# audiocogs/aac.js

Hardware: AMD Instinct MI355X
Metric: AAC-LC 48 kHz stereo frames/sec per node + achieved HBM GB/s vs roofline (higher is better)
Workload: dtype f32

## Files before the change

aac.js_amd/csrc/aacg_device.h:

```cpp
#ifndef AACG_DEVICE_H
#define AACG_DEVICE_H

#include <stdint.h>
#include "../../include/aacgpu.h"
#include "../../include/aacgpu_tools.h"

#define AACG_RUN_W        AACG_RUN_FRAMES
#define AACG_WG_WAVES     AACG_RUN_W
#define AACG_WG_THREADS   (AACG_WG_WAVES * 64)

#define AACG_PCM_SCALE (1.0f / 32768.0f)

struct aacg_c2 { float re, im; };

struct aacg_tables {
    aacg_c2 sincos_long[8][64];
    aacg_c2 tw512[7][64];
    aacg_c2 tw64[7][8];
    aacg_c2 sincos_short[8][8];
    float win_long[2][1024];
    float win_short[2][128];
    float sf[432];
    float iq_signed[1024];
    uint8_t band_of_long[1024];
    uint8_t band_of_short[128];
    float iq[8192];
};

#define AACG_TAB_OFF_SINCOS_LONG  0
#define AACG_TAB_OFF_TW512        (AACG_TAB_OFF_SINCOS_LONG + 8 * 64 * 2)
#define AACG_TAB_OFF_TW64         (AACG_TAB_OFF_TW512 + 7 * 64 * 2)
#define AACG_TAB_OFF_SINCOS_SHORT (AACG_TAB_OFF_TW64 + 7 * 8 * 2)
#define AACG_TAB_OFF_WIN_LONG     (AACG_TAB_OFF_SINCOS_SHORT + 8 * 8 * 2)
#define AACG_TAB_OFF_WIN_SHORT    (AACG_TAB_OFF_WIN_LONG + 2 * 1024)
#define AACG_TAB_F32_FLOATS       (AACG_TAB_OFF_WIN_SHORT + 2 * 128)
#define AACG_TAB_OFF_SF           AACG_TAB_F32_FLOATS
#define AACG_TAB_OFF_IQ_SMALL     (AACG_TAB_OFF_SF + 432)
#define AACG_TAB_OFF_BAND_LONG    (AACG_TAB_OFF_IQ_SMALL + 1024)
#define AACG_TAB_OFF_BAND_SHORT   (AACG_TAB_OFF_BAND_LONG + 256)
#define AACG_TAB_QUANT_FLOATS     (AACG_TAB_OFF_BAND_SHORT + 32)

#define AACG_SLOT_FLOATS  2048
#define AACG_TAB_SLOT_BASE(tab_floats) (((tab_floats) + 127) & ~127)
#define AACG_LDS_FLOATS(tab_floats) (AACG_TAB_SLOT_BASE(tab_floats) + AACG_WG_WAVES * AACG_SLOT_FLOATS + AACG_WG_WAVES)
#define AACG_LDS_BYTES_F32    (4 * AACG_LDS_FLOATS(AACG_TAB_F32_FLOATS))
#define AACG_LDS_BYTES_QUANT  (4 * AACG_LDS_FLOATS(AACG_TAB_QUANT_FLOATS))

struct aacg_dev_unit {
    aacg_unit_desc d;
    uint32_t gmap[2];
    uint32_t cpl_first, cpl_n;
};

struct aacg_dev_tns {
    int32_t start[8];
    int32_t size[8];
    int32_t inc[8];
    int32_t order[8];
    float   lpc[8][AACG_TNS_MAX_ORDER];
};

struct aacg_pns_tables {
    float    rnd[1024];
    double   esum[1028];
    uint16_t swb_long[64];
    uint16_t swb_short[16];
};

#define AACG_OV_BUFFERS 16
#define AACG_PIPE_STREAMS 3

struct aacg_run {
    int32_t pred_unit;
    int32_t n_units;
    int32_t is_last;
    uint32_t wave_nch;
    int32_t ov0[2];
    int32_t rot[2];
    int32_t unit[AACG_RUN_W];
    int32_t  wave_unit[AACG_RUN_W];
    uint32_t wave_coef[AACG_RUN_W];
    uint32_t wave_meta[AACG_RUN_W];
};
static_assert(sizeof(aacg_run) == 288 && __builtin_offsetof(aacg_run, ov0) == 16 && __builtin_offsetof(aacg_run, wave_unit) == 96,
              "aacg_run: the header is read as eight dwords, the per-wave words by offset (imdct_run_body)");
static inline int32_t aacg_run_wave_unit(const aacg_run& r, int w)
{
    if (r.pred_unit >= 0 && w == 0) return r.pred_unit;
    const int k = (r.pred_unit >= 0 && r.n_units < AACG_RUN_W) ? w - 1 : w;
    return k < r.n_units ? r.unit[k] : -1;
}

struct aacg_couple_job {
    uint32_t cce_unit;
    uint32_t src, dst, stride;
    uint32_t gain_off;
    uint32_t reserved[3];
};

struct aacg_couple_params {
    const aacg_couple_job* jobs;
    const aacg_dev_unit*   units;
    const aacg_band_meta*  meta;
    const aacg_tables*     tab;
    const float*           gains;
    float*                 spec;
    const float*           side;
    float*                 pcm;
    int32_t                n_jobs;
    int32_t                reserved;
};

struct aacg_kparams {
    const aacg_dev_unit*  units;
    const aacg_run*       runs;
    const void*           coeffs;
    const aacg_band_meta* meta;
    const aacg_dev_tns*   tns;
    float*                pcm;
    float*                overlap;
    float*                spec_out;
    const aacg_tables*    tab;
    int32_t               flip;
    int32_t               n_runs;
    int32_t               ablate;
    int32_t               reserved;
    float*                scratch;
    const aacg_pns_tables* pns;
};
static inline void aacg_set_tns_m(aacg_kparams* P, const double* m) { P->scratch = (float*)(void*)m; }
static inline void aacg_set_cpl(aacg_kparams* P, const aacg_couple_job* jobs, const float* gains, const float* side)
{
    P->scratch = (float*)(void*)jobs; P->pns = (const aacg_pns_tables*)(const void*)gains; P->spec_out = (float*)side;
}
#define AACG_CPL_JOBS(P)  ((const aacg_couple_job*)(const void*)(P).scratch)
#define AACG_CPL_GAINS(P) ((const float*)(const void*)(P).pns)
#define AACG_CPL_SIDE(P)  ((const float*)(P).spec_out)

struct aacg_rv_link {
    int32_t link_in;
    int32_t link_out;
    int32_t succ_unit;
    int32_t reserved;
};
#define AACG_RV_STATE_WORDS 2
#define AACG_RV_DATA_FLOATS 4096
#define AACG_RV_TAIL 1ull
#define AACG_RV_HEAD 2ull

struct aacg_xl_cell {
    unsigned long long state;
    unsigned long long pcm;
    uint32_t n_out_ch;
    uint32_t reserved[3];
};
struct aacg_rv_args {
    const aacg_rv_link*  links;
    unsigned long long*  state;
    float*               data;
    unsigned long long   epoch;
    aacg_xl_cell*        xl_cells;
    float*               xl_head;
    unsigned long long   epoch_in;
};

#define AACG_PARSE_WG_SMALL   256
#define AACG_PARSE_WG_LARGE   1024
#define AACG_PARSE_L1_BITS    9
#define AACG_PARSE_LUT_WORDS  12288
#define AACG_PARSE_BUCKETS    1024
#define AACG_PARSE_PAD_BYTES  32
#define AACG_PARSE_LDS_FIXED(lut_words, threads) ((size_t)(lut_words) * 4u + 160u + (size_t)AACG_MAX_SECTIONS * (threads) + 16u)
typedef struct aacg_parse_tables {
    uint32_t lut[AACG_PARSE_LUT_WORDS];
    uint32_t lut_words;
    uint16_t swb_long[64];
    uint16_t swb_short[16];
    uint32_t n_swb_long, n_swb_short;
    float    tns_coef[4][16];
} aacg_parse_tables;

typedef struct aacg_parse_params {
    const uint32_t* bytes;
    const aacg_parse_frame* frames;
    const aacg_parse_tables* tab;
    aacg_unit_desc* units;
    int16_t* q;
    aacg_band_meta* meta;
    aacg_tns_info* tns;
    aacg_parse_result* results;
    uint32_t n_frames, max_units, max_channels, options;
    uint32_t arena_bytes;
    uint32_t wg_threads;
    const uint32_t* order;
} aacg_parse_params;

typedef struct aacg_walk_params {
    aacg_parse_params P;
    aacg_parse_frame* blocks;
    aacg_walk_result* results;
    uint32_t max_frames;
} aacg_walk_params;

#endif
```

aac.js_amd/csrc/aacg_engine.hip:

```cpp
#include <hip/hip_runtime.h>

#include <chrono>
#include <hip/hip_ext.h>

#include <cstdio>
#include <cstdlib>
#include <cstring>
#include <new>
#include <string>
#include <algorithm>
#include <vector>
#include <mutex>
#include <thread>
#include <unordered_map>
#include <sys/mman.h>

#include "aacg_kernels.h"
#include "aacg_host.h"
#include "aacg_routes.h"
#include "aacg_wait.h"

extern "C" __global__ __launch_bounds__(AACG_WG_THREADS)
void aacg_imdct_run_quant(const aacg_kparams P) { imdct_run_body<AACG_INPUT_QUANT_I16>(P); }

// ... 5 lines not shown
    {0, "aacg_imdct_run_f32", (const void*)aacg_imdct_run_f32}
};
const int aacg_run_kernels_plain_n = 2;

void aacg_refresh_launch(aacg_dev_unit* units, const aacg_unit_desc* parsed, aacg_parse_result* results, const aacg_refresh_map* map, uint32_t n_units,
                         uint32_t max_units, int refuse_pns, uint32_t* refused, hipStream_t s);
int aacg_spectral_ex_set_lds_limits(void);
void aacg_spectral_ex_launch(bool quant, int n_units, hipStream_t s, const aacg_kparams& P);
void aacg_tns_matrices_launch(const aacg_dev_tns* d_recs, double* d_m, uint32_t n_records, hipStream_t s);
void aacg_couple_launch(bool pcm, hipStream_t s, const aacg_couple_params& Q);
struct cce_bufs { const aacg_run* runs; const aacg_couple_job* jobs; const float* gains; float* side; };
struct rv_bufs { const aacg_run* runs; const aacg_rv_link* links; unsigned long long* state; float* data; };

extern "C" __global__ __launch_bounds__(AACG_WG_THREADS)
void aacg_spectral(const aacg_kparams P, int n_units) { spectral_body(P, n_units); }

extern "C" __global__ void aacg_probe_wait(const unsigned* flag, unsigned* seen, long long ticks)
{
    const long long t0 = wall_clock64();
    unsigned ok = 0;
    while (!ok && wall_clock64() - t0 < ticks) ok = __hip_atomic_load(flag, __ATOMIC_RELAXED, __HIP_MEMORY_SCOPE_AGENT);
    *seen = ok;
}
extern "C" __global__ void aacg_probe_set(unsigned* flag) { __hip_atomic_store(flag, 1u, __ATOMIC_RELAXED, __HIP_MEMORY_SCOPE_AGENT); }

#define AACG_LDS_BYTES_SPECTRAL ((AACG_TAB_QUANT_FLOATS + AACG_WG_WAVES * 512) * 4)

struct aacg_engine {
    aacg_config cfg;
    hipStream_t stream = nullptr;
    aacg_tables* d_tab = nullptr;
    aacg_pns_tables* d_pns = nullptr;
    unsigned long long rv_epoch = 0;
    float* d_overlap = nullptr;
    std::vector<uint8_t> parity;
    uint64_t epoch = 0;
    aacg_tables h_tab;
    aacg_host_windows h_win;
    struct pipe_t {
        hipStream_t stream[AACG_PIPE_STREAMS] = {};
        hipEvent_t mark[AACG_PIPE_RING][AACG_PIPE_STREAMS] = {};
        hipEvent_t seen[AACG_PIPE_RING][AACG_PIPE_STREAMS] = {};
        hipEvent_t tail[AACG_PIPE_STREAMS] = {};
        hipEvent_t fork = nullptr;
        uint64_t n = 0;
        int streams = AACG_PIPE_STREAMS;
        uint64_t issued = 0;
        hipStream_t joined_stream = nullptr; uint64_t joined_n = ~0ull;
        bool open = false;
        bool concurrent = false;
        bool serial = false;
        aacg_plan* plan = nullptr;
        unsigned long long epoch = 0;
        uint64_t chained = 0;
    } pipe;
    aacg_xl_cell* d_xl_cells = nullptr;
    float* d_xl_head = nullptr;
    struct slot_t {
        hipStream_t stream = nullptr;
        hipEvent_t done = nullptr, kernel_done = nullptr;
        bool busy = false;
        void* d_units = nullptr;  size_t units_cap = 0;
        void* d_runs = nullptr;   size_t runs_cap = 0;
        void* d_coeffs = nullptr; size_t coeffs_cap = 0;
        void* d_meta = nullptr;   size_t meta_cap = 0;
        void* d_tns = nullptr;    size_t tns_cap = 0;
        void* d_scratch = nullptr; size_t scratch_cap = 0;
        void* d_spec = nullptr;   size_t spec_cap = 0;
        void* d_cce[4] = {nullptr, nullptr, nullptr, nullptr}; size_t cce_cap[4] = {0, 0, 0, 0};
        void* d_rv[4] = {nullptr, nullptr, nullptr, nullptr}; size_t rv_cap[4] = {0, 0, 0, 0};
        void* d_pcm = nullptr;    size_t pcm_cap = 0;
        void* h_in = nullptr;     size_t h_in_cap = 0;
        void* h_pcm = nullptr;    size_t h_pcm_cap = 0;
        void* user_pcm = nullptr; size_t user_pcm_bytes = 0;
        aacg_plan_host h;
    } slot[2];
    std::vector<std::pair<void*, size_t>> pool;
    uint64_t submitted = 0;
    hipEvent_t last_kernel = nullptr;
    void* d_trace = nullptr;
    int debug_route = 0;
    int ablate = 0;
    aacg_wait_policy wait;
    std::vector<hipStream_t> foreign;
    float* h_ov = nullptr;
    bool wedged = false;
    hipStream_t dump_stream = nullptr;
    aacg_xl_cell* h_dump = nullptr;
    std::string pipe_note;
    std::string err;
};

#define AACG_PLAN_BUFFERS 13
struct aacg_plan {
    aacg_engine* e;
    aacg_plan_host h;
    uint32_t n_units = 0;
    aacg_dev_unit* d_units = nullptr;
    aacg_run* d_runs = nullptr;
    aacg_dev_tns* d_tns = nullptr;
    float* d_scratch = nullptr;
    float* d_spec = nullptr;
    void*  d_cce[4] = {nullptr, nullptr, nullptr, nullptr};
    void*  d_rv[4] = {nullptr, nullptr, nullptr, nullptr};
    size_t bytes[AACG_PLAN_BUFFERS] = {0, 0, 0, 0, 0, 0, 0, 0, 0, 0, 0, 0, 0};
    hipEvent_t uploaded = nullptr;
    hipEvent_t last_use = nullptr;
    hipStream_t last_stream = nullptr;
    uint32_t unit_sets = 1, cur_set = 0;
    const aacg_dev_unit* units_now() const { return d_units + (size_t)cur_set * n_units; }
    bool used = false;
    bool last_pipelined = false;
    uint64_t seen_epoch = ~0ull;
    uint32_t launches = 0;
};

namespace {

bool hip_ok(aacg_engine* e, hipError_t rc, const char* what)
{
    if (rc == hipSuccess) return true;
    if (e) e->err = std::string(what) + ": " + hipGetErrorString(rc);
    return false;
}

#define HIP_TRY(e, call, code) do { if (!hip_ok((e), (call), #call)) return (code); } while (0)

size_t coef_elem_size(const aacg_engine* e) { return e->cfg.input_kind == AACG_INPUT_QUANT_I16 ? 2 : 4; }
size_t pcm_elem_size(const aacg_engine* e) { return e->cfg.output_kind == AACG_OUTPUT_I16 ? 2 : 4; }

void* pool_take(aacg_engine* e, size_t bytes, size_t* got)
{
    size_t best = e->pool.size();
    for (size_t i = 0; i < e->pool.size(); i++)
        if (e->pool[i].second >= bytes && e->pool[i].second <= 2 * bytes + 4096 && (best == e->pool.size() || e->pool[i].second < e->pool[best].second)) best = i;
    if (best != e->pool.size()) {
        void* p = e->pool[best].first;
        *got = e->pool[best].second;
        e->pool.erase(e->pool.begin() + (long)best);
        return p;
    }
    void* p = nullptr;
    if (!hip_ok(e, hipMalloc(&p, bytes), "hipMalloc (plan)")) return nullptr;
    *got = bytes;
    return p;
}

void pool_give(aacg_engine* e, void* p, size_t bytes)
{
    if (!p) return;
    if (e->pool.size() >= 48) { (void)hipFree(e->pool.front().first); e->pool.erase(e->pool.begin()); }
    e->pool.emplace_back(p, bytes);
}

int grow(aacg_engine* e, void** p, size_t* cap, size_t need)
{
    if (need <= *cap) return AACG_OK;
    if (*p) { (void)hipFree(*p); *p = nullptr; *cap = 0; }
    HIP_TRY(e, hipMalloc(p, need), AACG_ERR_OUT_OF_MEMORY);
    *cap = need;
    return AACG_OK;
}

int grow_host(aacg_engine* e, void** p, size_t* cap, size_t need)
{
    if (need <= *cap) return AACG_OK;
    if (*p) { (void)hipHostFree(*p); *p = nullptr; *cap = 0; }
    HIP_TRY(e, hipHostMalloc(p, need, hipHostMallocDefault), AACG_ERR_OUT_OF_MEMORY);
    *cap = need;
    return AACG_OK;
}

bool is_pinned(const void* p)
{
    hipPointerAttribute_t a;
    if (hipPointerGetAttributes(&a, p) != hipSuccess) { (void)hipGetLastError(); return false; }
    return a.type == hipMemoryTypeHost;
}

#define AACG_DUMP_CELLS 4096u
const char* event_state(hipEvent_t ev)
{
    if (!ev) return "-";
    const hipError_t st = hipEventQuery(ev);
    (void)hipGetLastError();
    return st == hipSuccess ? "done" : st == hipErrorNotReady ? "PENDING" : "error";
}
const char* stream_state(hipStream_t s)
{
    const hipError_t st = hipStreamQuery(s);
    (void)hipGetLastError();
    return st == hipSuccess ? "idle" : st == hipErrorNotReady ? "BUSY" : "error";
}

std::string in_flight(aacg_engine* e)
{
    char b[512];
    std::string o;
    const aacg_engine::pipe_t& pp = e->pipe;
    std::snprintf(b, sizeof b, "pipeline: %llu launches issued, %llu in the current sequence on %d streams, %llu chained, open %d serial %d concurrent %d, rv epoch %llu; ",
                  (unsigned long long)pp.issued, (unsigned long long)pp.n, pp.streams, (unsigned long long)pp.chained, (int)pp.open, (int)pp.serial, (int)pp.concurrent, e->rv_epoch);
    o += b;
    o += std::string("engine stream ") + stream_state(e->stream);
    for (int k = 0; k < AACG_PIPE_STREAMS; k++) if (pp.stream[k]) { std::snprintf(b, sizeof b, ", pipe stream %d %s", k, stream_state(pp.stream[k])); o += b; }
    for (int k = 0; k < 2; k++) if (e->slot[k].stream) { std::snprintf(b, sizeof b, ", batch slot %d %s (busy %d, kernel %s, copy-back %s)", k, stream_state(e->slot[k].stream), (int)e->slot[k].busy, event_state(e->slot[k].kernel_done), event_state(e->slot[k].done)); o += b; }
    for (size_t k = 0; k < e->foreign.size(); k++) { std::snprintf(b, sizeof b, ", caller stream %p %s", (void*)e->foreign[k], stream_state(e->foreign[k])); o += b; }
    if (pp.stream[0]) {
        o += "; completion events [ring slot: per stream]";
        for (int r = 0; r < AACG_PIPE_RING; r++) {
            std::snprintf(b, sizeof b, " %d:", r); o += b;
            for (int k = 0; k < AACG_PIPE_STREAMS; k++) { o += k ? "/" : ""; o += event_state(pp.seen[r][k] ? pp.seen[r][k] : nullptr); }
        }
    }
    const size_t n_cells = (size_t)e->cfg.max_streams * (size_t)e->cfg.max_channels * (size_t)AACG_OV_BUFFERS;
    const size_t take = n_cells < AACG_DUMP_CELLS ? n_cells : AACG_DUMP_CELLS;
    if (!e->dump_stream && hipStreamCreateWithFlags(&e->dump_stream, hipStreamNonBlocking) != hipSuccess) { (void)hipGetLastError(); e->dump_stream = nullptr; }
    hipStream_t ds = e->dump_stream;
    aacg_xl_cell* h = e->h_dump;
    if (e->d_xl_cells && ds && h && hipMemcpyAsync(h, e->d_xl_cells, take * sizeof(aacg_xl_cell), hipMemcpyDeviceToHost, ds) == hipSuccess) {
        aacg_wait_policy quick; quick.limit_s = 0.25;
        if (aacg_wait_stream(ds, quick) == hipSuccess) {
            unsigned long long n_tail = 0, n_head = 0, lo = ~0ull, hi = 0;
            std::string heads;
            for (size_t i = 0; i < take; i++) {
                const unsigned long long w = h[i].state, ep = w >> 2;
                if (!w) continue;
                if ((w & 3) == AACG_RV_TAIL) n_tail++;
                if ((w & 3) == AACG_RV_HEAD) { n_head++; if (n_head <= 4) { std::snprintf(b, sizeof b, " cell %zu epoch %llu", i, ep); heads += b; } }
                lo = ep < lo ? ep : lo; hi = ep > hi ? ep : hi;
            }
            std::snprintf(b, sizeof b, "; cross-launch cells (first %zu of %zu): %llu TAIL, %llu HEAD (a HEAD nobody finished = a consumer whose producer never came:%s), epochs %llu..%llu",
                          take, n_cells, n_tail, n_head, heads.empty() ? " none" : heads.c_str(), lo == ~0ull ? 0ull : lo, hi);
            o += b;
        } else o += "; cross-launch cells unreadable: a device-to-host copy on a fresh stream did not complete in 250 ms either";
    } else { (void)hipGetLastError(); o += "; cross-launch cells not read"; }
    return o;
}

int timed_out(aacg_engine* e, const char* what)
{
    char b[160];
    std::snprintf(b, sizeof b, "%s: the GPU did not answer within %.1f s (aacg_set_wait_limit_ms). In flight: ", what, e->wait.limit_s);
    e->err = std::string(b) + in_flight(e);
    e->wedged = true;
    return AACG_ERR_TIMEOUT;
}
int wait_stream(aacg_engine* e, hipStream_t s, const char* what)
{
    const hipError_t st = aacg_wait_stream(s, e->wait);
    if (st == hipSuccess) return AACG_OK;
    if (st == hipErrorNotReady) return timed_out(e, what);
    e->err = std::string(what) + ": " + hipGetErrorString(st);
    return AACG_ERR_NO_DEVICE;
}
int wait_event(aacg_engine* e, hipEvent_t ev, const char* what)
{
    const hipError_t st = aacg_wait_event(ev, e->wait);
    if (st == hipSuccess) return AACG_OK;
    if (st == hipErrorNotReady) return timed_out(e, what);
    e->err = std::string(what) + ": " + hipGetErrorString(st);
    return AACG_ERR_NO_DEVICE;
}
void note_stream(aacg_engine* e, hipStream_t s)
{
    if (!s || s == e->stream) return;
    for (hipStream_t k : e->pipe.stream) if (k == s) return;
    for (hipStream_t k : e->foreign) if (k == s) return;
    if (e->foreign.size() >= 32) e->foreign.erase(e->foreign.begin());
    e->foreign.push_back(s);
}

}

const aacg_run_kernel* aacg_find_run_kernel(unsigned key)
{
    const aacg_run_kernel* const tabs[] = {aacg_run_kernels_plain, aacg_run_kernels_rv, aacg_run_kernels_nt, aacg_run_kernels_ext,
                                           aacg_run_kernels_i16, aacg_run_kernels_exrun, aacg_run_kernels_couple};
    const int counts[] = {aacg_run_kernels_plain_n, aacg_run_kernels_rv_n, aacg_run_kernels_nt_n, aacg_run_kernels_ext_n,
                          aacg_run_kernels_i16_n, aacg_run_kernels_exrun_n, aacg_run_kernels_couple_n};
    for (size_t t = 0; t < sizeof tabs / sizeof tabs[0]; t++)
        for (int i = 0; i < counts[t]; i++)
            if (tabs[t][i].key == key) return &tabs[t][i];
    return nullptr;
}

namespace {

aacg_route route_of(const aacg_engine* e, const aacg_plan_host& h, bool pipelined)
{
    return aacg_pick_route(e->cfg.input_kind, e->cfg.output_kind, e->debug_route, e->d_trace != nullptr, h, pipelined);
}

bool needs_spec_buffer(const aacg_engine* e, const aacg_plan_host& h) { return route_of(e, h, false).stage != AACG_STAGE_NONE; }

int launch_kernel(aacg_engine* e, const aacg_run_kernel* k, unsigned blocks, hipStream_t s, const aacg_kparams& P, const aacg_rv_args* V, hipEvent_t stop = nullptr)
{
    if (!k) { e->err = "no run kernel for this route"; return AACG_ERR_UNSUPPORTED; }
    aacg_kparams p = P;
    aacg_rv_args v;
    void* args[8] = {&p, nullptr, nullptr, nullptr, nullptr, nullptr, nullptr, nullptr};
    if (k->key & AACG_RK_RV) { v = *V; args[1] = &v; }
    const void *a_runs = p.runs, *a_tab = p.tab, *a_links = V ? V->links : nullptr, *a_units = p.units, *a_coeffs = p.coeffs, *a_meta = p.meta;
    if (k->preloaded) { args[0] = &a_runs; args[1] = &a_tab; args[2] = &a_links; args[3] = &a_units; args[4] = &a_coeffs; args[5] = &a_meta; args[6] = &p; args[7] = &v; }
    const dim3 block(AACG_WG_THREADS);
    if (stop) HIP_TRY(e, hipExtLaunchKernel(k->fn, dim3(blocks), block, args, 0, s, nullptr, stop, 0), AACG_ERR_NO_DEVICE);
    else      HIP_TRY(e, hipLaunchKernel(k->fn, dim3(blocks), block, args, 0, s), AACG_ERR_NO_DEVICE);
    return AACG_OK;
}

static size_t tns_record_bytes(size_t n) { return (sizeof(aacg_dev_tns) * n + 255u) & ~(size_t)255u; }
static size_t tns_buffer_bytes(size_t n) { return n ? tns_record_bytes(n) + sizeof(double) * AACG_TNS_M_DOUBLES * n : 0; }
static double* tns_matrices_of(const aacg_dev_tns* d_tns, size_t n) { return (double*)((char*)const_cast<aacg_dev_tns*>(d_tns) + tns_record_bytes(n)); }

struct xl_args { bool on; unsigned long long epoch_in; int set; int trace_part = 0; };

int launch_run(aacg_engine* e, const aacg_route& R, const aacg_dev_unit* d_units, const aacg_run* d_runs, const aacg_dev_tns* d_tns,
               float* d_scratch, float* d_spec, const cce_bufs& cb, const rv_bufs& rvb, const aacg_plan_host& h, const void* d_coeffs, const aacg_band_meta* d_meta,
               void* d_pcm, int flip, hipStream_t s, const xl_args& xl, unsigned long long* epoch_out, hipEvent_t stop = nullptr)
{
    if (h.zero_fill)
        HIP_TRY(e, hipMemsetAsync(d_pcm, 0, h.pcm_floats * pcm_elem_size(e), s), AACG_ERR_NO_DEVICE);
    aacg_kparams P;
    std::memset(&P, 0, sizeof P);
    P.units = d_units; P.coeffs = d_coeffs; P.meta = d_meta; P.pcm = (float*)d_pcm;
    P.overlap = e->d_overlap; P.tab = e->d_tab; P.flip = flip;
    if (R.rv) {
        const size_t n_runs = h.runs_rv.size(), n_links = h.n_links_rv;
        P.runs = rvb.runs; P.n_runs = (int32_t)n_runs;
        aacg_rv_args V;
        std::memset(&V, 0, sizeof V);
        V.links = rvb.links;
        V.state = rvb.state ? rvb.state + (size_t)xl.set * AACG_RV_STATE_WORDS * n_links : nullptr;
        V.data = rvb.data ? rvb.data + (size_t)xl.set * AACG_RV_DATA_FLOATS * n_links : nullptr;
        V.epoch = ++e->rv_epoch;
        if (xl.on) { V.xl_cells = e->d_xl_cells; V.xl_head = e->d_xl_head; V.epoch_in = xl.epoch_in; }
        if (R.run_key & AACG_RK_EX) {
            P.tns = h.any_tns ? d_tns : nullptr; P.pns = e->d_pns;
            if (h.any_tns) aacg_set_tns_m(&P, tns_matrices_of(d_tns, h.tns.size()));
        }
        if (epoch_out) *epoch_out = V.epoch;
        P.ablate = e->d_trace ? e->ablate : (e->ablate & ~16);
        if (e->d_trace) P.spec_out = (float*)e->d_trace + (size_t)xl.trace_part * (1u << 18);
        return launch_kernel(e, aacg_find_run_kernel(R.run_key), (unsigned)n_runs, s, P, &V, stop);
    }
    P.runs = d_runs; P.n_runs = (int32_t)h.runs.size();
    P.tns = h.any_tns ? d_tns : nullptr;
    P.scratch = h.needs_scratch ? d_scratch : nullptr;
    P.ablate = e->d_trace ? e->ablate : (e->ablate & ~16);
    if (e->d_trace) P.spec_out = (float*)e->d_trace;
    auto couple = [&](int point) {
        for (uint32_t r = 0; r < h.couple_rounds; r++) {
            const uint32_t first = h.couple_first[(size_t)point * h.couple_rounds + r], last = h.couple_first[(size_t)point * h.couple_rounds + r + 1];
            if (last <= first) continue;
            aacg_couple_params Q;
            Q.jobs = cb.jobs + first; Q.n_jobs = (int32_t)(last - first); Q.units = d_units; Q.meta = d_meta; Q.tab = e->d_tab;
            Q.gains = cb.gains; Q.spec = d_spec; Q.side = cb.side; Q.pcm = (float*)d_pcm; Q.reserved = 0;
            aacg_couple_launch(point == AACG_CCE_AFTER_IMDCT, s, Q);
        }
    };
    if (R.stage == AACG_STAGE_DEPENDENT_COUPLING) {
        float* trace_or_null = P.spec_out;
        P.spec_out = d_spec; P.pns = e->d_pns; P.tns = nullptr;
        if (R.stage_quant) aacg_spectral_ex_launch(true, (int)h.units.size(), s, P);
        else HIP_TRY(e, hipMemcpyAsync(d_spec, d_coeffs, (size_t)h.coef_blocks * 4096u, hipMemcpyDeviceToDevice, s), AACG_ERR_NO_DEVICE);
        couple(AACG_CCE_BEFORE_TNS);
        if (h.any_tns) {
            P.coeffs = d_spec; P.meta = nullptr; P.tns = d_tns;
            { aacg_kparams Q = P; aacg_set_tns_m(&Q, tns_matrices_of(d_tns, h.tns.size())); aacg_spectral_ex_launch(false, (int)h.units.size(), s, Q); }
        }
        couple(AACG_CCE_AFTER_TNS);
        P.spec_out = trace_or_null; P.coeffs = d_spec; P.meta = nullptr; P.tns = nullptr;
    } else if (R.stage == AACG_STAGE_SPECTRAL_EX) {
        float* trace_or_null = P.spec_out;
        P.spec_out = d_spec; P.pns = e->d_pns;
        { aacg_kparams Q = P; if (h.any_tns) aacg_set_tns_m(&Q, tns_matrices_of(d_tns, h.tns.size())); aacg_spectral_ex_launch(R.stage_quant, (int)h.units.size(), s, Q); }
        P.spec_out = trace_or_null; P.coeffs = d_spec; P.meta = nullptr; P.tns = nullptr;
    } else if (R.has_run && (R.run_key & AACG_RK_EX)) {
        P.pns = e->d_pns;
        if (h.any_tns) aacg_set_tns_m(&P, tns_matrices_of(d_tns, h.tns.size()));
    }
    int rc = AACG_OK;
    auto side_pass = [&]() {
        aacg_kparams C = P;
        C.runs = cb.runs; C.n_runs = (int32_t)h.cce_runs.size(); C.pcm = cb.side; C.scratch = nullptr;
        return launch_kernel(e, aacg_find_run_kernel(R.side_key), (unsigned)h.cce_runs.size(), s, C, nullptr);
    };
    if (R.has_side && R.side_first && (rc = side_pass())) return rc;
    if (R.has_run) {
        if (R.run_key & AACG_RK_CPL) aacg_set_cpl(&P, cb.jobs + h.fused_first, cb.gains, cb.side);
        if ((rc = launch_kernel(e, aacg_find_run_kernel(R.run_key), (unsigned)h.runs.size(), s, P, nullptr))) return rc;
    }
    if (R.has_side && !R.side_first && (rc = side_pass())) return rc;
    if (R.couple_pcm) couple(AACG_CCE_AFTER_IMDCT);
    HIP_TRY(e, hipGetLastError(), AACG_ERR_NO_DEVICE);
    return AACG_OK;
}

int pipe_join(aacg_engine* e, hipStream_t s)
{
    aacg_engine::pipe_t& pp = e->pipe;
    if (!pp.open) return AACG_OK;
    if (s && s == pp.joined_stream && pp.issued == pp.joined_n) return AACG_OK;
    for (int k = 0; k < AACG_PIPE_STREAMS; k++) {
        if (s == pp.stream[k]) continue;
        if (s) {
            HIP_TRY(e, hipEventRecord(pp.tail[k], pp.stream[k]), AACG_ERR_NO_DEVICE);
            HIP_TRY(e, hipStreamWaitEvent(s, pp.tail[k], 0), AACG_ERR_NO_DEVICE);
        } else { const int wrc = wait_stream(e, pp.stream[k], "waiting for the pipelined launches"); if (wrc) return wrc; }
    }
    if (!s) pp.open = false;
    pp.joined_stream = s; pp.joined_n = pp.issued;
    return AACG_OK;
}

int quiesce(aacg_engine* e, const char* what)
{
    int rc = wait_stream(e, e->stream, what);
    if (rc) return rc;
    if (e->pipe.stream[0]) {
        for (hipStream_t ps : e->pipe.stream) if (ps && (rc = wait_stream(e, ps, what))) return rc;
        e->pipe.open = false;
        e->pipe.joined_stream = nullptr; e->pipe.joined_n = e->pipe.issued;
    }
    for (auto& sl : e->slot) if (sl.stream && (rc = wait_stream(e, sl.stream, what))) return rc;
    for (size_t k = 0; k < e->foreign.size();) {
        const hipError_t st = aacg_wait_stream(e->foreign[k], e->wait);
        if (st == hipErrorNotReady) return timed_out(e, what);
        if (st != hipSuccess) { (void)hipGetLastError(); e->foreign.erase(e->foreign.begin() + (long)k); continue; }
        k++;
    }
    e->wedged = false;
    return AACG_OK;
}

}

extern "C" {

int aacg_abi_version(void) { return AACG_ABI_VERSION; }

const char* aacg_kernel_name(void) { return "aacg_imdct_run_quant_rv"; }

int aacg_debug_set_route(aacg_engine* e, int flags)
{
    if (!e || (flags & ~(AACG_DEBUG_ROUTE_UNFUSED_COUPLING | AACG_DEBUG_ROUTE_RECOMPUTE))) return AACG_ERR_INVALID_ARG;
    e->debug_route = flags;
    return AACG_OK;
}

int aacg_plan_kernels(aacg_engine* e, const aacg_plan* p, char* dst, size_t n)
{
    return aacg_plan_kernels_ex(e, p, 0, dst, n);
}

int aacg_plan_kernels_ex(aacg_engine* e, const aacg_plan* p, int pipelined, char* dst, size_t n)
{
    if (!e || !p || p->e != e || !dst || n == 0) return AACG_ERR_INVALID_ARG;
    const std::string r = aacg_route_names(route_of(e, p->h, pipelined != 0), p->h.any_tns);
    if (r.size() + 1 > n) return AACG_ERR_INVALID_ARG;
    std::memcpy(dst, r.c_str(), r.size() + 1);
    return AACG_OK;
}

int aacg_debug_route(int input_kind, int output_kind, int debug_route, int plan_flags, int pipelined, char* dst, size_t n)
{
    if (!dst || n == 0) return AACG_ERR_INVALID_ARG;
    aacg_plan_host h;
    h.any_tns = (plan_flags & AACG_ROUTE_PLAN_TNS) != 0;
    h.any_pns = (plan_flags & AACG_ROUTE_PLAN_PNS) != 0;
    h.needs_scratch = (plan_flags & AACG_ROUTE_PLAN_FULL_LATER_RUNS) != 0;
    h.long_chains = (plan_flags & (AACG_ROUTE_PLAN_LONG_CHAINS | AACG_ROUTE_PLAN_FULL_LATER_RUNS)) != 0;
    h.wide_frames = (plan_flags & AACG_ROUTE_PLAN_WIDE_FRAMES) != 0;
    h.any_cce = (plan_flags & (AACG_ROUTE_PLAN_CCE_INDEPENDENT | AACG_ROUTE_PLAN_CCE_DEPENDENT)) != 0;
    h.any_cce_dependent = (plan_flags & AACG_ROUTE_PLAN_CCE_DEPENDENT) != 0;
    h.fused_independent = (plan_flags & AACG_ROUTE_PLAN_CCE_INDEPENDENT) && !h.needs_scratch;
    if (plan_flags & AACG_ROUTE_PLAN_CCE_INDEPENDENT) h.cce_runs.resize(1);
    if (!(plan_flags & AACG_ROUTE_PLAN_NO_RUNS)) { h.runs.resize(1); h.runs_rv.resize(1); }
    const aacg_route r = aacg_pick_route(input_kind, output_kind, debug_route, false, h, pipelined != 0);
    if ((r.has_run && !aacg_find_run_kernel(r.run_key)) || (r.has_side && !aacg_find_run_kernel(r.side_key))) return AACG_ERR_UNSUPPORTED;
    const std::string t = aacg_route_names(r, h.any_tns);
    if (t.size() + 1 > n) return AACG_ERR_INVALID_ARG;
    std::memcpy(dst, t.c_str(), t.size() + 1);
    return AACG_OK;
}

int aacg_debug_pipeline_order(unsigned long long n, int streams, int* stream, long long* sync_round, int* marked, long long* complete_upto)
{
    const aacg_pipe_order o = aacg_pipeline_order(n, streams);
    if (stream) *stream = o.stream;
    if (sync_round) *sync_round = o.sync_round;
    if (marked) *marked = o.marked ? 1 : 0;
    if (complete_upto) *complete_upto = o.complete_upto;
    return AACG_OV_BUFFERS;
}

int aacg_debug_run_kernel(int index, char* dst, size_t n)
{
    const aacg_run_kernel* const tabs[] = {aacg_run_kernels_plain, aacg_run_kernels_rv, aacg_run_kernels_nt, aacg_run_kernels_ext,
                                           aacg_run_kernels_i16, aacg_run_kernels_exrun, aacg_run_kernels_couple};
    const int counts[] = {aacg_run_kernels_plain_n, aacg_run_kernels_rv_n, aacg_run_kernels_nt_n, aacg_run_kernels_ext_n,
                          aacg_run_kernels_i16_n, aacg_run_kernels_exrun_n, aacg_run_kernels_couple_n};
    for (size_t t = 0; t < sizeof tabs / sizeof tabs[0]; t++) {
        if (index < counts[t]) {
            if (!dst || std::strlen(tabs[t][index].name) + 1 > n) return AACG_ERR_INVALID_ARG;
            std::strcpy(dst, tabs[t][index].name);
            return (int)tabs[t][index].key;
        }
        index -= counts[t];
    }
    return AACG_ERR_INVALID_ARG;
}

const char* aacg_last_error(const aacg_engine* e) { return e ? e->err.c_str() : "null engine"; }

int aacg_create(const aacg_config* cfg, aacg_engine** out)
{
    if (!cfg || !out) return AACG_ERR_INVALID_ARG;
    *out = nullptr;
    if (cfg->abi_version != AACG_ABI_VERSION || cfg->max_streams < 1 || cfg->max_channels < 1 ||
        cfg->max_channels > AACG_MAX_CHANNELS || (cfg->tns_mode != AACG_TNS_REFERENCE && cfg->tns_mode != AACG_TNS_SPEC) ||
        (cfg->pns_mode != AACG_PNS_REFERENCE && cfg->pns_mode != AACG_PNS_SPEC) ||
        (cfg->pns_mode == AACG_PNS_SPEC && cfg->input_kind != AACG_INPUT_QUANT_I16) ||
        (cfg->output_kind != AACG_OUTPUT_F32 && cfg->output_kind != AACG_OUTPUT_I16) ||
        (cfg->cce_mode != AACG_CCE_REFERENCE && cfg->cce_mode != AACG_CCE_SPEC) ||
        (cfg->cce_mode == AACG_CCE_SPEC && cfg->output_kind != AACG_OUTPUT_F32) ||
        (cfg->input_kind != AACG_INPUT_SPEC_F32 && cfg->input_kind != AACG_INPUT_QUANT_I16))
        return AACG_ERR_INVALID_ARG;

    int n_dev = 0;
    if (hipGetDeviceCount(&n_dev) != hipSuccess || cfg->device_ordinal < 0 || cfg->device_ordinal >= n_dev)
        return AACG_ERR_NO_DEVICE;

    aacg_engine* e = new (std::nothrow) aacg_engine();
    if (!e) return AACG_ERR_OUT_OF_MEMORY;
    e->cfg = *cfg;
    int rc = aacg_build_tables(cfg->sample_index, &e->h_tab, &e->h_win);
    if (rc) { delete e; return rc; }

    const size_t n_cells = (size_t)cfg->max_streams * (size_t)cfg->max_channels * (size_t)AACG_OV_BUFFERS;
    const size_t ov_bytes = n_cells * 1024u * sizeof(float);
    if (!hip_ok(e, hipSetDevice(cfg->device_ordinal), "hipSetDevice") ||
        !hip_ok(e, hipStreamCreateWithFlags(&e->stream, hipStreamNonBlocking), "hipStreamCreate") ||
        !hip_ok(e, hipMalloc((void**)&e->d_tab, sizeof(aacg_tables)), "hipMalloc tables") ||
        !hip_ok(e, hipMalloc((void**)&e->d_overlap, ov_bytes), "hipMalloc overlap") ||
        !hip_ok(e, hipMemcpy(e->d_tab, &e->h_tab, sizeof(aacg_tables), hipMemcpyHostToDevice), "upload tables") ||
        !hip_ok(e, hipMemset(e->d_overlap, 0, ov_bytes), "zero overlap") ||
        !hip_ok(e, hipMalloc((void**)&e->d_xl_cells, n_cells * sizeof(aacg_xl_cell)), "hipMalloc cells") ||
        !hip_ok(e, hipMemset(e->d_xl_cells, 0, n_cells * sizeof(aacg_xl_cell)), "zero cells") ||
        !hip_ok(e, hipMalloc((void**)&e->d_xl_head, ov_bytes), "hipMalloc heads") ||
        aacg_spectral_ex_set_lds_limits() != 0 ||
        !hip_ok(e, hipFuncSetAttribute((const void*)aacg_spectral, hipFuncAttributeMaxDynamicSharedMemorySize, AACG_LDS_BYTES_SPECTRAL), "LDS attr")) {
        std::fprintf(stderr, "aacgpu: %s\n", e->err.c_str());
        aacg_destroy(e);
        return AACG_ERR_NO_DEVICE;
    }
    e->parity.assign((size_t)cfg->max_streams * (size_t)cfg->max_channels, 0);
    for (int i = 0;; i++) {
        char name[96];
        const int key = aacg_debug_run_kernel(i, name, sizeof name);
        if (key < 0) break;
        if (aacg_run_kernel_name((unsigned)key) != name) { std::fprintf(stderr, "aacgpu: run kernel table: %s registered with switches %d\n", name, key); aacg_destroy(e); return AACG_ERR_INVALID_ARG; }
    }
    if (cfg->pns_mode == AACG_PNS_SPEC) {
        aacg_pns_tables* pt = new (std::nothrow) aacg_pns_tables;
        const bool ok = pt && aacg_build_pns_tables(cfg->sample_index, pt) == AACG_OK &&
                        hip_ok(e, hipMalloc((void**)&e->d_pns, sizeof *pt), "hipMalloc pns tables") &&
                        hip_ok(e, hipMemcpy(e->d_pns, pt, sizeof *pt, hipMemcpyHostToDevice), "upload pns tables");
        delete pt;
        if (!ok) { aacg_destroy(e); return AACG_ERR_OUT_OF_MEMORY; }
    }
#ifdef AACG_PROFILE
    if (const char* a = std::getenv("AACG_ABLATE")) e->ablate = std::atoi(a);
    if ((e->ablate & 16) && hipMalloc(&e->d_trace, 1u << 22) == hipSuccess) (void)hipMemset(e->d_trace, 0, 1u << 22);
#endif
    if (!hip_ok(e, hipHostMalloc((void**)&e->h_ov, 4096, hipHostMallocDefault), "hipHostMalloc (overlap staging)") ||
        !hip_ok(e, hipHostMalloc((void**)&e->h_dump, AACG_DUMP_CELLS * sizeof(aacg_xl_cell), hipHostMallocDefault), "hipHostMalloc (dump staging)")) { aacg_destroy(e); return AACG_ERR_OUT_OF_MEMORY; }
    { const int wrc = wait_stream(e, nullptr, "aacg_create: waiting for the table uploads"); if (wrc) { std::fprintf(stderr, "aacgpu: %s\n", e->err.c_str()); aacg_destroy(e); return wrc; } }
    *out = e;
    return AACG_OK;
}

int aacg_set_wait_limit_ms(aacg_engine* e, uint32_t ms)
{
    if (!e || !ms) return AACG_ERR_INVALID_ARG;
    e->wait.limit_s = ms * 1e-3;
    return AACG_OK;
}
int aacg_debug_in_flight(aacg_engine* e, char* dst, size_t n)
{
    if (!e || !dst || !n) return AACG_ERR_INVALID_ARG;
    (void)hipSetDevice(e->cfg.device_ordinal);
    const std::string t = in_flight(e);
    std::snprintf(dst, n, "%s", t.c_str());
    return (int)t.size();
}
static int pipe_setup(aacg_engine* e);
int aacg_debug_stall(aacg_engine* e, int which, uint32_t ms)
{
    if (!e || which < 0 || which > AACG_PIPE_STREAMS || ms > 5000) return AACG_ERR_INVALID_ARG;
    HIP_TRY(e, hipSetDevice(e->cfg.device_ordinal), AACG_ERR_NO_DEVICE);
    if (which) { const int rc = pipe_setup(e); if (rc) return rc; }
    hipStream_t s = which ? e->pipe.stream[which - 1] : e->stream;
    static unsigned* d_flag = nullptr;
    if (!d_flag) { HIP_TRY(e, hipMalloc((void**)&d_flag, 8), AACG_ERR_OUT_OF_MEMORY); HIP_TRY(e, hipMemset(d_flag, 0, 8), AACG_ERR_NO_DEVICE); }
    hipLaunchKernelGGL(aacg_probe_wait, dim3(1), dim3(1), 0, s, d_flag, d_flag + 1, (long long)ms * 100000LL);
    HIP_TRY(e, hipGetLastError(), AACG_ERR_NO_DEVICE);
    if (which) { e->pipe.open = true; e->pipe.issued++; }
// ... 801 lines not shown
```

aac.js_amd/csrc/aacg_engine_rv.hip:

```cpp
#include <hip/hip_runtime.h>

#include "aacg_kernels.h"
#include "aacg_routes.h"

AACG_RUN_KERNEL_PRE(aacg_imdct_run_quant_rv, AACG_INPUT_QUANT_I16, AACG_OUTPUT_F32, false, false, false, true, false)
AACG_RUN_KERNEL_PRE(aacg_imdct_run_f32_rv, AACG_INPUT_SPEC_F32, AACG_OUTPUT_F32, false, false, false, true, false)
AACG_RUN_KERNEL_PRE(aacg_imdct_run_quant_rv_nt, AACG_INPUT_QUANT_I16, AACG_OUTPUT_F32, false, false, false, true, true)
AACG_RUN_KERNEL_PRE(aacg_imdct_run_f32_rv_nt, AACG_INPUT_SPEC_F32, AACG_OUTPUT_F32, false, false, false, true, true)

const aacg_run_kernel aacg_run_kernels_rv[] = {
    {AACG_RK_RV | AACG_RK_QUANT, "aacg_imdct_run_quant_rv", (const void*)aacg_imdct_run_quant_rv, true},
    {AACG_RK_RV, "aacg_imdct_run_f32_rv", (const void*)aacg_imdct_run_f32_rv, true},
    {AACG_RK_RV | AACG_RK_NT | AACG_RK_QUANT, "aacg_imdct_run_quant_rv_nt", (const void*)aacg_imdct_run_quant_rv_nt, true},
    {AACG_RK_RV | AACG_RK_NT, "aacg_imdct_run_f32_rv_nt", (const void*)aacg_imdct_run_f32_rv_nt, true}
};
const int aacg_run_kernels_rv_n = 4;
```

aac.js_amd/csrc/aacg_kernels.h:

```cpp
#ifndef AACG_KERNELS_H
#define AACG_KERNELS_H

#include "devport.h"
#include "aacg_device.h"

#ifdef AACG_PROFILE
#define AACG_ABL(P, bits) ((P).ablate & (bits))
#else
#define AACG_ABL(P, bits) 0
#endif

struct cpx { float re, im; };

DP_DEVICE cpx c_add(cpx a, cpx b) { cpx r; r.re = a.re + b.re; r.im = a.im + b.im; return r; }
DP_DEVICE cpx c_sub(cpx a, cpx b) { cpx r; r.re = a.re - b.re; r.im = a.im - b.im; return r; }
DP_DEVICE cpx c_muli(cpx a)       { cpx r; r.re = -a.im; r.im = a.re; return r; }
DP_DEVICE cpx c_mul(cpx a, cpx w)
{
#pragma clang fp contract(off)
    cpx r;
    r.re = dp_fma(a.re, w.re, -(a.im * w.im));
    r.im = dp_fma(a.re, w.im, a.im * w.re);
    return r;
}

DP_DEVICE void radix8_inv(cpx (&x)[8])
{
#pragma clang fp contract(off)
    const float h = 0.70710678118654752440f;
    cpx a0 = c_add(x[0], x[4]), a1 = c_sub(x[0], x[4]);
    cpx a2 = c_add(x[2], x[6]), a3 = c_sub(x[2], x[6]);
    cpx a4 = c_add(x[1], x[5]), a5 = c_sub(x[1], x[5]);
    cpx a6 = c_add(x[3], x[7]), a7 = c_sub(x[3], x[7]);
    cpx e0 = c_add(a0, a2), e2 = c_sub(a0, a2);
    cpx ia3 = c_muli(a3), ia7 = c_muli(a7);
    cpx e1 = c_add(a1, ia3), e3 = c_sub(a1, ia3);
    cpx o0 = c_add(a4, a6), o2 = c_sub(a4, a6);
    cpx o1 = c_add(a5, ia7), o3 = c_sub(a5, ia7);
    cpx t1, t2, t3;
    t1.re = (o1.re - o1.im) * h;  t1.im = (o1.re + o1.im) * h;
    t2 = c_muli(o2);
    t3.re = -(o3.re + o3.im) * h; t3.im = (o3.re - o3.im) * h;
    x[0] = c_add(e0, o0); x[4] = c_sub(e0, o0);
    x[1] = c_add(e1, t1); x[5] = c_sub(e1, t1);
    x[2] = c_add(e2, t2); x[6] = c_sub(e2, t2);
    x[3] = c_add(e3, t3); x[7] = c_sub(e3, t3);
}

DP_DEVICE dpv2 k8_ld2(const float* p) { const dpf2 t = *(const dpf2*)p; dpv2 r; r[0] = t.x; r[1] = t.y; return r; }
DP_DEVICE void k8_st2(float* p, dpv2 v) { dpf2 t; t.x = v[0]; t.y = v[1]; *(dpf2*)p = t; }
DP_DEVICE dpv2 k8_v2(float a, float b) { dpv2 r; r[0] = a; r[1] = b; return r; }

DP_DEVICE void k8_radix8(dpv2 (&x)[8])
{
    const dpv2 h = {0.70710678118654752440f, 0.70710678118654752440f};
    const dpv2 mh = {-0.70710678118654752440f, -0.70710678118654752440f};
    const dpv2 a0 = x[0] + x[4], a1 = x[0] - x[4], a2 = x[2] + x[6], a3 = x[2] - x[6];
    const dpv2 a4 = x[1] + x[5], a5 = x[1] - x[5], a6 = x[3] + x[7], a7 = x[3] - x[7];
    const dpv2 e0 = a0 + a2, e2 = a0 - a2, e1 = dp_cadd_i(a1, a3), e3 = dp_csub_i(a1, a3);
    const dpv2 o0 = a4 + a6, o2 = a4 - a6, o1 = dp_cadd_i(a5, a7), o3 = dp_csub_i(a5, a7);
    const dpv2 s1 = dp_cadd_i(o1, o1);
    const dpv2 s3 = dp_cadd_i(-o3, o3);
    x[0] = e0 + o0; x[4] = e0 - o0;
    x[1] = dp_fma2(s1, h, e1); x[5] = dp_fma2(s1, mh, e1);
    x[2] = dp_cadd_i(e2, o2); x[6] = dp_csub_i(e2, o2);
    x[3] = dp_fma2(s3, h, e3); x[7] = dp_fma2(s3, mh, e3);
}

DP_DEVICE void lds_put(float* base, int idx, cpx v)
{
    dpf2 t; t.x = v.re; t.y = v.im;
    *(dpf2*)(base + 2 * idx) = t;
}
DP_DEVICE cpx lds_get(const float* base, int idx)
{
    dpf2 t = *(const dpf2*)(base + 2 * idx);
    cpx v; v.re = t.x; v.im = t.y; return v;
}

struct unit_view {
    uint32_t pcm_offset, coef_offset, meta_offset, tns_offset;
    int channel, n_out_ch, n_ch, flags;
    int seq[2], shape[2], shape_prev[2], max_sfb[2], tns[2];
    uint32_t gmap[2];
    uint32_t cpl_first, cpl_n;
};
DP_DEVICE unit_view load_unit(const aacg_dev_unit* u)
{
    const uint32_t* w = (const uint32_t*)u;
    unit_view v;
    const uint32_t w2 = w[2], w3 = w[3];
    v.pcm_offset = w[1]; v.coef_offset = w[4]; v.meta_offset = w[5];
    v.channel = (int)(w2 & 0xffffu); v.n_out_ch = (int)(w2 >> 16);
    v.n_ch = (int)(w3 & 0xffu); v.flags = (int)((w3 >> 8) & 0xffu);
#pragma unroll
    for (int c = 0; c < 2; c++) {
        const uint32_t ci = w[6 + 4 * c], cj = w[7 + 4 * c];
        v.seq[c] = (int)(ci & 0xffu); v.shape[c] = (int)((ci >> 8) & 0xffu);
        v.shape_prev[c] = (int)((ci >> 16) & 0xffu); v.max_sfb[c] = (int)(ci >> 24);
        v.tns[c] = (int)((cj >> 8) & AACG_CHAN_TNS_PRESENT);
        v.gmap[c] = w[16 + c];
    }
    v.tns_offset = w[14];
    v.cpl_first = w[18]; v.cpl_n = w[19];
    return v;
}

DP_DEVICE void stage_tables_load(const aacg_tables* T, int n_floats, dpf4& t0, dpf4& t1)
{
    const dpf4* src = (const dpf4*)T;
    const int n4 = n_floats >> 2, tid = dp_tid();
    const int i1 = tid + AACG_WG_THREADS;
    t0 = src[tid < n4 ? tid : n4 - 1];
    t1 = src[i1 < n4 ? i1 : n4 - 1];
}
DP_DEVICE void stage_tables_store(float* lds, int n_floats, const dpf4& t0, const dpf4& t1)
{
    dpf4* dst = (dpf4*)lds;
    const int n4 = n_floats >> 2, tid = dp_tid();
    if (tid < n4) dst[tid] = t0;
    if (tid + AACG_WG_THREADS < n4) dst[tid + AACG_WG_THREADS] = t1;
}
DP_DEVICE void stage_tables(const aacg_tables* T, float* lds, int n_floats)
{
    dpf4 t0, t1;
    stage_tables_load(T, n_floats, t0, t1);
    stage_tables_store(lds, n_floats, t0, t1);
}

DP_DEVICE dpf2 head_window(const float* tab, int seq, int shape_prev, int n)
{
    const float* wl = tab + AACG_TAB_OFF_WIN_LONG + 1024 * shape_prev;
    if (seq != AACG_LONG_STOP_SEQUENCE) return *(const dpf2*)(wl + n);
    const float* ws = tab + AACG_TAB_OFF_WIN_SHORT + 128 * shape_prev;
    int i = n - 448; i = i < 0 ? 0 : (i > 126 ? 126 : i);
    dpf2 v = *(const dpf2*)(ws + i);
    if (n < 448) { v.x = 0.0f; v.y = 0.0f; }
    if (n >= 576) { v.x = AACG_PCM_SCALE; v.y = AACG_PCM_SCALE; }
    return v;
}
DP_DEVICE dpf2 tail_window(const float* tab, int seq, int shape, int n)
{
    dpf2 v, r;
    if (seq != AACG_LONG_START_SEQUENCE) {
        v = *(const dpf2*)(tab + AACG_TAB_OFF_WIN_LONG + 1024 * shape + 1022 - n);
        r.x = v.y; r.y = v.x;
        return r;
    }
    int i = 574 - n; i = i < 0 ? 0 : (i > 126 ? 126 : i);
    v = *(const dpf2*)(tab + AACG_TAB_OFF_WIN_SHORT + 128 * shape + i);
    r.x = v.y; r.y = v.x;
    if (n < 448) { r.x = AACG_PCM_SCALE; r.y = AACG_PCM_SCALE; }
    if (n >= 576) { r.x = 0.0f; r.y = 0.0f; }
    return r;
}

DP_DEVICE void wfix(float& r, float w) { r = (w == 0.0f) ? 0.0f : r; }

DP_DEVICE int xch1(int q, int l)     { return 64 * q + (l ^ (q << 3)); }
DP_DEVICE int xch2(int row, int col) { return 8 * row + (col ^ ((row >> 2) & 7)); }

struct chan_par { int seq, shape, shape_prev; };

DP_DEVICE int long_col(int l);

template <int SEQ>
DP_DEVICE void long_planar_window(const float* tab, const chan_par& cp, bool want_head, float* area, int l ,
                                  const float (&R)[8], const float (&I)[8], const float (&m)[16],
                                  float (&hx)[8], float (&hy)[8])
{
#pragma clang fp contract(off)
#pragma unroll
    for (int j = 0; j < 4; j++) {
        const int n = 2 * l + 128 * j;
        const dpf2 w0 = head_window(tab, SEQ, cp.shape_prev, n), w1 = head_window(tab, SEQ, cp.shape_prev, n + 512);
        const dpf2 v0 = tail_window(tab, SEQ, cp.shape, n), v1 = tail_window(tab, SEQ, cp.shape, n + 512);
        if (want_head) {
            hx[j]     = I[j + 4] * w0.x;
            hy[j]     = -m[3 - j] * w0.y;
            hx[j + 4] = R[j] * w1.x;
            hy[j + 4] = -m[8 + 7 - j] * w1.y;
            if (SEQ == AACG_LONG_STOP_SEQUENCE) { wfix(hx[j], w0.x); wfix(hy[j], w0.y); wfix(hx[j + 4], w1.x); wfix(hy[j + 4], w1.y); }
        }
        dpf2 t, t2;
        t.x = R[j + 4] * v0.x;
        t.y = -m[8 + 3 - j] * v0.y;
        t2.x = -I[j] * v1.x;
        t2.y = m[7 - j] * v1.y;
        if (SEQ == AACG_LONG_START_SEQUENCE) { wfix(t.x, v0.x); wfix(t.y, v0.y); wfix(t2.x, v1.x); wfix(t2.y, v1.y); }
        *(dpf2*)(area + n) = t;
        *(dpf2*)(area + n + 512) = t2;
    }
}

template <int NC, bool VM = false>
DP_DEVICE void long_channels(const float* tab, const chan_par (&cp)[NC], bool want_head,
                             float* const (&area)[NC], float (&hx)[NC][8], float (&hy)[NC][8])
{
#pragma clang fp contract(off)
    const int l = dp_lane();
    const float* sincos = tab + AACG_TAB_OFF_SINCOS_LONG;

    dpv2 z[NC][8];
#pragma unroll
    for (int j = 0; j < 8; j++) {
        const dpv2 sc = k8_ld2(sincos + 2 * (64 * j + l));
#pragma unroll
        for (int c = 0; c < NC; c++) {
            const dpf2 a = *(const dpf2*)(area[c] + 2 * l + 128 * j);
            const dpf2 b = *(const dpf2*)(area[c] + 1022 - 2 * l - 128 * j);
            z[c][j] = dp_cmul(k8_v2(b.y, a.x), sc);
        }
    }
    dp_wave_sync();

#pragma unroll
    for (int c = 0; c < NC; c++) k8_radix8(z[c]);
#pragma unroll
    for (int q = 1; q < 8; q++) {
        const dpv2 tw = k8_ld2(tab + AACG_TAB_OFF_TW512 + 2 * (64 * (q - 1) + l));
#pragma unroll
        for (int c = 0; c < NC; c++) z[c][q] = dp_cmul(z[c][q], tw);
    }
#pragma unroll
    for (int q = 0; q < 8; q++)
#pragma unroll
        for (int c = 0; c < NC; c++) k8_st2(area[c] + 2 * xch1(q, l), z[c][q]);
    dp_wave_sync();
    const int l0 = l & 7, qq = l >> 3;
#pragma unroll
    for (int j = 0; j < 8; j++)
#pragma unroll
        for (int c = 0; c < NC; c++) z[c][j] = k8_ld2(area[c] + 2 * xch1(qq, l0 + 8 * j));
    dp_wave_sync();
#pragma unroll
    for (int c = 0; c < NC; c++) k8_radix8(z[c]);
#pragma unroll
    for (int r = 1; r < 8; r++) {
        const dpv2 tw = k8_ld2(tab + AACG_TAB_OFF_TW64 + 2 * (8 * (r - 1) + l0));
#pragma unroll
        for (int c = 0; c < NC; c++) z[c][r] = dp_cmul(z[c][r], tw);
    }
#pragma unroll
    for (int r = 0; r < 8; r++)
#pragma unroll
        for (int c = 0; c < NC; c++) k8_st2(area[c] + 2 * xch2(qq + 8 * r, l0), z[c][r]);
    dp_wave_sync();
    const int col = VM ? long_col(l) : l;
#pragma unroll
    for (int i = 0; i < 8; i++)
#pragma unroll
        for (int c = 0; c < NC; c++) z[c][i] = k8_ld2(area[c] + 2 * xch2(col, i));
    dp_wave_sync();
#pragma unroll
    for (int c = 0; c < NC; c++) k8_radix8(z[c]);

    float R[NC][8], I[NC][8];
#pragma unroll
    for (int r = 0; r < 8; r++) {
        const dpv2 sc = k8_ld2(sincos + 2 * (64 * r + col));
#pragma unroll
        for (int c = 0; c < NC; c++) {
            const dpv2 ri = dp_cmul(z[c][r], sc);
            R[c][r] = ri[0]; I[c][r] = ri[1];
        }
    }

#pragma unroll
    for (int c = 0; c < NC; c++) {
        float m[16], own[16];
#pragma unroll
        for (int r = 0; r < 8; r++) { own[r] = m[r] = R[c][r]; own[8 + r] = m[8 + r] = I[c][r]; }
        if (VM) dp_mirror16_valu(own, m); else dp_shfl(m, 63 - l);
        if (cp[c].seq == AACG_ONLY_LONG_SEQUENCE)       long_planar_window<AACG_ONLY_LONG_SEQUENCE>(tab, cp[c], want_head, area[c], col, R[c], I[c], m, hx[c], hy[c]);
        else if (cp[c].seq == AACG_LONG_START_SEQUENCE) long_planar_window<AACG_LONG_START_SEQUENCE>(tab, cp[c], want_head, area[c], col, R[c], I[c], m, hx[c], hy[c]);
        else                                            long_planar_window<AACG_LONG_STOP_SEQUENCE>(tab, cp[c], want_head, area[c], col, R[c], I[c], m, hx[c], hy[c]);
    }
}
template <int NC, bool VM = false>
DP_DEVICE void short_channels(const float* tab, const chan_par (&cp)[NC],
                              float* const (&area)[NC], float (&hx)[NC][8], float (&hy)[NC][8])
{
#pragma clang fp contract(off)
    const int l = dp_lane(), w = l >> 3, g = l & 7;
    const float* sincos = tab + AACG_TAB_OFF_SINCOS_SHORT;

    dpv2 z[NC][8];
#pragma unroll
    for (int j = 0; j < 8; j++) {
        const dpv2 sc = k8_ld2(sincos + 2 * (8 * j + g));
#pragma unroll
        for (int c = 0; c < NC; c++) {
            const dpf2 a = *(const dpf2*)(area[c] + 128 * w + 2 * g + 16 * j);
            const dpf2 b = *(const dpf2*)(area[c] + 128 * w + 126 - 2 * g - 16 * j);
            z[c][j] = dp_cmul(k8_v2(b.y, a.x), sc);
        }
    }
    dp_wave_sync();

#pragma unroll
    for (int c = 0; c < NC; c++) k8_radix8(z[c]);
#pragma unroll
    for (int q = 1; q < 8; q++) {
        const dpv2 tw = k8_ld2(tab + AACG_TAB_OFF_TW64 + 2 * (8 * (q - 1) + g));
#pragma unroll
        for (int c = 0; c < NC; c++) z[c][q] = dp_cmul(z[c][q], tw);
    }
#pragma unroll
    for (int q = 0; q < 8; q++)
#pragma unroll
        for (int c = 0; c < NC; c++) k8_st2(area[c] + 2 * xch2(8 * w + q, g), z[c][q]);
    dp_wave_sync();
#pragma unroll
    for (int i = 0; i < 8; i++)
#pragma unroll
        for (int c = 0; c < NC; c++) z[c][i] = k8_ld2(area[c] + 2 * xch2(l, i));
    dp_wave_sync();
#pragma unroll
    for (int c = 0; c < NC; c++) k8_radix8(z[c]);

    float R[NC][8], I[NC][8];
#pragma unroll
    for (int r = 0; r < 8; r++) {
        const dpv2 sc = k8_ld2(sincos + 2 * (8 * r + g));
#pragma unroll
        for (int c = 0; c < NC; c++) {
            const dpv2 ri = dp_cmul(z[c][r], sc);
            R[c][r] = ri[0]; I[c][r] = ri[1];
        }
    }

#pragma unroll
    for (int c = 0; c < NC; c++) {
        float m[16], own[16];
#pragma unroll
        for (int r = 0; r < 8; r++) { own[r] = m[r] = R[c][r]; own[8 + r] = m[8 + r] = I[c][r]; }
        if (VM) dp_mirror8_valu(own, m); else dp_shfl(m, l ^ 7);

        const float* ws = tab + AACG_TAB_OFF_WIN_SHORT + 128 * cp[c].shape;
        const float* wh = (w == 0) ? tab + AACG_TAB_OFF_WIN_SHORT + 128 * cp[c].shape_prev : ws;
        float hd[16], tl[16];
#pragma unroll
        for (int j = 0; j < 4; j++) {
            const int i = 2 * g + 16 * j;
            const dpf2 h0 = *(const dpf2*)(wh + i), h1 = *(const dpf2*)(wh + i + 64);
            const dpf2 t0 = *(const dpf2*)(ws + 126 - i), t1 = *(const dpf2*)(ws + 62 - i);
            hd[j]         = I[c][j + 4] * h0.x;
            hd[8 + j]     = -m[3 - j] * h0.y;
            hd[j + 4]     = R[c][j] * h1.x;
            hd[8 + j + 4] = -m[8 + 7 - j] * h1.y;
            tl[j]         = R[c][j + 4] * t0.y;
            tl[8 + j]     = -m[8 + 3 - j] * t0.x;
            tl[j + 4]     = -I[c][j] * t1.y;
            tl[8 + j + 4] = m[7 - j] * t1.x;
        }
        float pt[16];
#pragma unroll
        for (int i = 0; i < 16; i++) pt[i] = tl[i];
        dp_shfl(pt, (l - 8) & 63);
#pragma unroll
        for (int i = 0; i < 8; i++) {
            hx[c][i] = (w == 0 ? 0.0f : pt[i]) + hd[i];
            hy[c][i] = (w == 0 ? 0.0f : pt[8 + i]) + hd[8 + i];
        }

        float* tail = area[c];
#pragma unroll
        for (int mm = 0; mm < 8; mm++) {
            const int p = 128 * w + 2 * g + 16 * mm;
            if (p >= 576) { dpf2 t; t.x = hx[c][mm]; t.y = hy[c][mm]; *(dpf2*)(tail + p - 576) = t; }
            if (w == 7)   { dpf2 t; t.x = tl[mm]; t.y = tl[8 + mm]; *(dpf2*)(tail + 448 + 2 * g + 16 * mm) = t; }
        }
#pragma unroll
        for (int t4 = 0; t4 < 4; t4++) {
            const int n = 576 + 2 * l + 128 * t4;
            if (n < 1024) { dpf2 zz; zz.x = 0.0f; zz.y = 0.0f; *(dpf2*)(tail + n) = zz; }
        }
    }
}

DP_DEVICE int stg(int k);

struct cpx2 { dpv2 re, im; };

DP_DEVICE dpv2 v2(float a, float b) { dpv2 r; r[0] = a; r[1] = b; return r; }
DP_DEVICE dpv2 v2s(float s) { dpv2 r; r[0] = s; r[1] = s; return r; }
DP_DEVICE void wfix2(dpv2& r, float w) { r = (w == 0.0f) ? v2s(0.0f) : r; }
DP_DEVICE cpx2 c2_add(cpx2 a, cpx2 b) { cpx2 r; r.re = a.re + b.re; r.im = a.im + b.im; return r; }
DP_DEVICE cpx2 c2_sub(cpx2 a, cpx2 b) { cpx2 r; r.re = a.re - b.re; r.im = a.im - b.im; return r; }
DP_DEVICE cpx2 c2_muli(cpx2 a) { cpx2 r; r.re = -a.im; r.im = a.re; return r; }
DP_DEVICE cpx2 c2_mul(cpx2 a, cpx w)
{
    cpx2 r;
    const dpv2 wr = v2s(w.re), wi = v2s(w.im);
    r.re = a.re * wr - a.im * wi;
    r.im = a.re * wi + a.im * wr;
    return r;
}

DP_DEVICE void radix8_inv2(cpx2 (&x)[8])
{
    const dpv2 h = v2s(0.70710678118654752440f);
    cpx2 a0 = c2_add(x[0], x[4]), a1 = c2_sub(x[0], x[4]);
    cpx2 a2 = c2_add(x[2], x[6]), a3 = c2_sub(x[2], x[6]);
    cpx2 a4 = c2_add(x[1], x[5]), a5 = c2_sub(x[1], x[5]);
    cpx2 a6 = c2_add(x[3], x[7]), a7 = c2_sub(x[3], x[7]);
    cpx2 e0 = c2_add(a0, a2), e2 = c2_sub(a0, a2);
    cpx2 ia3 = c2_muli(a3), ia7 = c2_muli(a7);
    cpx2 e1 = c2_add(a1, ia3), e3 = c2_sub(a1, ia3);
    cpx2 o0 = c2_add(a4, a6), o2 = c2_sub(a4, a6);
    cpx2 o1 = c2_add(a5, ia7), o3 = c2_sub(a5, ia7);
    cpx2 t1, t2, t3;
    t1.re = (o1.re - o1.im) * h;  t1.im = (o1.re + o1.im) * h;
    t2 = c2_muli(o2);
    t3.re = -(o3.re + o3.im) * h; t3.im = (o3.re - o3.im) * h;
    x[0] = c2_add(e0, o0); x[4] = c2_sub(e0, o0);
    x[1] = c2_add(e1, t1); x[5] = c2_sub(e1, t1);
    x[2] = c2_add(e2, t2); x[6] = c2_sub(e2, t2);
    x[3] = c2_add(e3, t3); x[7] = c2_sub(e3, t3);
}

DP_DEVICE int pch1(int q, int l)     { return 64 * q + (l ^ (((q >> 1) & 1) << 3)); }
DP_DEVICE int pch2(int row, int col) { return 8 * row + (col ^ ((row >> 1) & 7)); }
DP_DEVICE void lds_put2(float* base, int slot, cpx2 v)
{
// ... 34 lines not shown
template <int SEQ>
DP_DEVICE void long_pair_window(const float* tab, const chan_par& cp, bool want_head, float* slot, int l ,
                                const dpv2 (&R)[8], const dpv2 (&I)[8], const dpv2 (&mR)[8], const dpv2 (&mI)[8],
                                dpv2 (&hx)[8], dpv2 (&hy)[8])
{
#pragma unroll
    for (int j = 0; j < 4; j++) {
        const int n = 2 * l + 128 * j;
        const dpf2 w0 = head_window(tab, SEQ, cp.shape_prev, n), w1 = head_window(tab, SEQ, cp.shape_prev, n + 512);
        const dpf2 v0 = tail_window(tab, SEQ, cp.shape, n), v1 = tail_window(tab, SEQ, cp.shape, n + 512);
        if (want_head) {
            hx[j]     = I[j + 4] * v2s(w0.x);
            hy[j]     = -mR[3 - j] * v2s(w0.y);
            hx[j + 4] = R[j] * v2s(w1.x);
            hy[j + 4] = -mI[7 - j] * v2s(w1.y);
            if (SEQ == AACG_LONG_STOP_SEQUENCE) { wfix2(hx[j], w0.x); wfix2(hy[j], w0.y); wfix2(hx[j + 4], w1.x); wfix2(hy[j + 4], w1.y); }
        }
        dpv2 t0 = R[j + 4] * v2s(v0.x), t1 = -mI[3 - j] * v2s(v0.y);
        dpv2 t2 = -I[j] * v2s(v1.x),    t3 = mR[7 - j] * v2s(v1.y);
        if (SEQ == AACG_LONG_START_SEQUENCE) { wfix2(t0, v0.x); wfix2(t1, v0.y); wfix2(t2, v1.x); wfix2(t3, v1.y); }
        dpf4 o;
        o.x = t0[0]; o.y = t0[1]; o.z = t1[0]; o.w = t1[1];
        *(dpf4*)(slot + 2 * n) = o;
        o.x = t2[0]; o.y = t2[1]; o.z = t3[0]; o.w = t3[1];
        *(dpf4*)(slot + 2 * (n + 512)) = o;
    }
}

template <bool VM>
DP_DEVICE void long_pair(const float* tab, const chan_par& cp, bool want_head, float* slot,
                         dpv2 (&hx)[8], dpv2 (&hy)[8])
{
    const int l = dp_lane();
    const float* sincos = tab + AACG_TAB_OFF_SINCOS_LONG;

    cpx2 z[8];
    {
        int eb[4], ob[4];
#pragma unroll
        for (int m = 0; m < 4; m++) { eb[m] = l ^ (m << 3); ob[m] = (63 - l) ^ ((3 - m) << 3); }
#pragma unroll
        for (int j = 0; j < 8; j++) {
            const cpx sc = lds_get(sincos, 64 * j + l);
            const dpv2 xe = lds_pair(slot, 64 * j + eb[j & 3]);
            const dpv2 xo = lds_pair(slot, 512 + 64 * (7 - j) + ob[j & 3]);
            z[j].im = xe * v2s(sc.re) + xo * v2s(sc.im);
            z[j].re = xo * v2s(sc.re) - xe * v2s(sc.im);
        }
    }
    dp_wave_sync();

    radix8_inv2(z);
#pragma unroll
    for (int q = 1; q < 8; q++) z[q] = c2_mul(z[q], lds_get(tab + AACG_TAB_OFF_TW512, 64 * (q - 1) + l));
    {
        const int w0 = l, w1 = l ^ 8;
#pragma unroll
        for (int q = 0; q < 8; q++) lds_put2(slot, 64 * q + ((q & 2) ? w1 : w0), z[q]);
    }
    dp_wave_sync();
    const int l0 = l & 7, qq = l >> 3;
    {
        const int q1 = (qq >> 1) & 1, r0 = 64 * qq + l0 + 8 * q1, r1 = 64 * qq + l0 - 8 * q1;
#pragma unroll
        for (int j = 0; j < 8; j++) z[j] = lds_get2(slot, ((j & 1) ? r1 : r0) + 8 * j);
    }
    dp_wave_sync();
    radix8_inv2(z);
#pragma unroll
    for (int r = 1; r < 8; r++) z[r] = c2_mul(z[r], lds_get(tab + AACG_TAB_OFF_TW64, 8 * (r - 1) + l0));
    {
        const int e0 = 8 * qq + (l0 ^ (qq >> 1)), e1 = e0 ^ 4;
#pragma unroll
        for (int r = 0; r < 8; r++) lds_put2(slot, 64 * r + ((r & 1) ? e1 : e0), z[r]);
    }
    dp_wave_sync();
    const int c = VM ? long_col(l) : l;
    {
        const int ab = dp_lds_addr(slot) + 16 * (8 * c + ((c >> 1) & 7));
#pragma unroll
        for (int i = 0; i < 8; i++) {
            const dpf4 t = dp_lds_read_f4(ab ^ (16 * i));
            z[i].re = v2(t.x, t.y); z[i].im = v2(t.z, t.w);
        }
    }
    dp_wave_sync();
    radix8_inv2(z);

    dpv2 R[8], I[8], mR[8], mI[8];
#pragma unroll
    for (int r = 0; r < 8; r++) {
        const cpx sc = lds_get(sincos, 64 * r + c);
        R[r] = z[r].re * v2s(sc.re) - z[r].im * v2s(sc.im);
        I[r] = z[r].im * v2s(sc.re) + z[r].re * v2s(sc.im);
    }
    if (cp.seq == AACG_ONLY_LONG_SEQUENCE) {
        dp_keep_branch();
        const float* wh = tab + AACG_TAB_OFF_WIN_LONG + 1024 * cp.shape_prev;
        const float* wt = tab + AACG_TAB_OFF_WIN_LONG + 1024 * cp.shape;
#pragma unroll
        for (int j = 0; j < 4; j++) {
            const int n = 2 * c + 128 * j;
            const dpf2 w0 = *(const dpf2*)(wh + n), w1 = *(const dpf2*)(wh + n + 512);
            const dpf2 r0 = *(const dpf2*)(wt + 1022 - n), r1 = *(const dpf2*)(wt + 510 - n);
            hx[j]     = I[j + 4] * v2s(w0.x);
            hx[j + 4] = R[j] * v2s(w1.x);
            const dpv2 t0 = R[j + 4] * v2s(r0.y), t2 = -I[j] * v2s(r1.y);
            dpv2 t1, t3;
            if (VM) {
                const float src[8] = {R[3 - j][0], R[3 - j][1], I[7 - j][0], I[7 - j][1], I[3 - j][0], I[3 - j][1], R[7 - j][0], R[7 - j][1]};
                const float wv[4] = {w0.y, w1.y, r0.x, r1.x};
                float o[8];
                dp_window_mirror<16>(src, wv, o, j == 0);
                hy[j] = v2(o[0], o[1]); hy[j + 4] = v2(o[2], o[3]); t1 = v2(o[4], o[5]); t3 = v2(o[6], o[7]);
            } else {
                if (j == 0) shfl_pairs<0>(R, I, 63 - l, mR, mI);
                hy[j]     = -mR[3 - j] * v2s(w0.y);
                hy[j + 4] = -mI[7 - j] * v2s(w1.y);
                t1 = -mI[3 - j] * v2s(r0.x); t3 = mR[7 - j] * v2s(r1.x);
            }
            dpf4 o;
            o.x = t0[0]; o.y = t0[1]; o.z = t1[0]; o.w = t1[1];
            *(dpf4*)(slot + 2 * n) = o;
            o.x = t2[0]; o.y = t2[1]; o.z = t3[0]; o.w = t3[1];
            *(dpf4*)(slot + 2 * (n + 512)) = o;
        }
        return;
    }
    shfl_pairs<VM ? 16 : 0>(R, I, 63 - l, mR, mI);
    if (cp.seq == AACG_LONG_START_SEQUENCE) long_pair_window<AACG_LONG_START_SEQUENCE>(tab, cp, want_head, slot, c, R, I, mR, mI, hx, hy);
    else                                    long_pair_window<AACG_LONG_STOP_SEQUENCE>(tab, cp, want_head, slot, c, R, I, mR, mI, hx, hy);
}

template <bool VM>
DP_DEVICE void short_pair(const float* tab, const chan_par& cp, float* slot, dpv2 (&hx)[8], dpv2 (&hy)[8])
{
    const int l = dp_lane(), w = l >> 3, g = l & 7;
    const float* sincos = tab + AACG_TAB_OFF_SINCOS_SHORT;

    cpx2 z[8];
    {
        const int w3 = (w & 3) << 3, e0 = ((w << 6) | g) | w3, o0 = (512 + ((w << 6) | (7 - g))) | w3;
        int eb[4], ob[4];
#pragma unroll
        for (int m = 0; m < 4; m++) { eb[m] = e0 ^ (m << 3); ob[m] = o0 ^ (m << 3); }
#pragma unroll
        for (int j = 0; j < 8; j++) {
            const cpx sc = lds_get(sincos, 8 * j + g);
            const dpv2 xe = lds_pair(slot, eb[j & 3] + 32 * (j >> 2));
            const dpv2 xo = lds_pair(slot, ob[3 - (j & 3)] + 32 * (1 - (j >> 2)));
            z[j].im = xe * v2s(sc.re) + xo * v2s(sc.im);
            z[j].re = xo * v2s(sc.re) - xe * v2s(sc.im);
        }
    }
    dp_wave_sync();

    radix8_inv2(z);
#pragma unroll
    for (int q = 1; q < 8; q++) z[q] = c2_mul(z[q], lds_get(tab + AACG_TAB_OFF_TW64, 8 * (q - 1) + g));
    {
        const int p0 = (w << 6) | (g ^ ((w & 1) << 2));
        int pb[4];
#pragma unroll
        for (int m = 0; m < 4; m++) pb[m] = p0 ^ m;
#pragma unroll
        for (int q = 0; q < 8; q++) lds_put2(slot, pb[q >> 1] + 8 * q, z[q]);
    }
    dp_wave_sync();
    {
        const int ab = dp_lds_addr(slot) + 16 * (8 * l + ((l >> 1) & 7));
#pragma unroll
        for (int i = 0; i < 8; i++) {
            const dpf4 t = dp_lds_read_f4(ab ^ (16 * i));
            z[i].re = v2(t.x, t.y); z[i].im = v2(t.z, t.w);
        }
    }
    dp_wave_sync();
    radix8_inv2(z);

    dpv2 R[8], I[8], mR[8], mI[8];
#pragma unroll
    for (int r = 0; r < 8; r++) {
        const cpx sc = lds_get(sincos, 8 * r + g);
        R[r] = z[r].re * v2s(sc.re) - z[r].im * v2s(sc.im);
        I[r] = z[r].im * v2s(sc.re) + z[r].re * v2s(sc.im);
    }
    if (!VM) shfl_pairs<0>(R, I, l ^ 7, mR, mI);

    const float* ws = tab + AACG_TAB_OFF_WIN_SHORT + 128 * cp.shape;
    const float* wh = (w == 0) ? tab + AACG_TAB_OFF_WIN_SHORT + 128 * cp.shape_prev : ws;
    dpv2 hd[16], tl[16];
#pragma unroll
    for (int j = 0; j < 4; j++) {
        const int i = 2 * g + 16 * j;
        const dpf2 h0 = *(const dpf2*)(wh + i), h1 = *(const dpf2*)(wh + i + 64);
        const dpf2 t0 = *(const dpf2*)(ws + 126 - i), t1 = *(const dpf2*)(ws + 62 - i);
        hd[j]         = I[j + 4] * v2s(h0.x);
        hd[j + 4]     = R[j] * v2s(h1.x);
        tl[j]         = R[j + 4] * v2s(t0.y);
        tl[j + 4]     = -I[j] * v2s(t1.y);
        if (VM) {
            const float src[8] = {R[3 - j][0], R[3 - j][1], I[7 - j][0], I[7 - j][1], I[3 - j][0], I[3 - j][1], R[7 - j][0], R[7 - j][1]};
            const float wv[4] = {h0.y, h1.y, t0.x, t1.x};
            float o[8];
            dp_window_mirror<8>(src, wv, o, j == 0);
            hd[8 + j] = v2(o[0], o[1]); hd[8 + j + 4] = v2(o[2], o[3]); tl[8 + j] = v2(o[4], o[5]); tl[8 + j + 4] = v2(o[6], o[7]);
        } else {
            hd[8 + j]     = -mR[3 - j] * v2s(h0.y);
            hd[8 + j + 4] = -mI[7 - j] * v2s(h1.y);
            tl[8 + j]     = -mI[3 - j] * v2s(t0.x);
            tl[8 + j + 4] = mR[7 - j] * v2s(t1.x);
        }
    }
    dpv2 pt[16];
#pragma unroll
    for (int m = 0; m < 8; m++) {
        dpf4 o; o.x = tl[2 * m][0]; o.y = tl[2 * m][1]; o.z = tl[2 * m + 1][0]; o.w = tl[2 * m + 1][1];
        *(dpf4*)(slot + 256 * m + 4 * l) = o;
    }
    dp_wave_sync();
    if (VM) {
#pragma unroll
        for (int m = 0; m < 16; m++) pt[m] = v2s(0.0f);
        if (w != 0) {
#pragma unroll
            for (int m = 0; m < 8; m++) {
                const dpf4 t = *(const dpf4*)(slot + 256 * m + 4 * (l - 8));
                pt[2 * m] = v2(t.x, t.y); pt[2 * m + 1] = v2(t.z, t.w);
            }
        }
    } else {
#pragma unroll
        for (int m = 0; m < 8; m++) {
            const dpf4 t = *(const dpf4*)(slot + 256 * m + 4 * ((l - 8) & 63));
            pt[2 * m] = v2(t.x, t.y); pt[2 * m + 1] = v2(t.z, t.w);
        }
    }
    dp_wave_sync();
#pragma unroll
    for (int i = 0; i < 8; i++) {
        hx[i] = ((!VM && w == 0) ? v2s(0.0f) : pt[i]) + hd[i];
        hy[i] = ((!VM && w == 0) ? v2s(0.0f) : pt[8 + i]) + hd[8 + i];
    }

    if (w >= 4) {
#pragma unroll
        for (int mm = 4; mm < 8; mm++) {
            const int p = 128 * w + 2 * g + 16 * mm;
            dpf4 o; o.x = hx[mm][0]; o.y = hx[mm][1]; o.z = hy[mm][0]; o.w = hy[mm][1]; *(dpf4*)(slot + 2 * (p - 576)) = o;
        }
    }
    if (w >= 5) {
#pragma unroll
        for (int mm = 0; mm < 4; mm++) {
            const int p = 128 * w + 2 * g + 16 * mm;
            dpf4 o; o.x = hx[mm][0]; o.y = hx[mm][1]; o.z = hy[mm][0]; o.w = hy[mm][1]; *(dpf4*)(slot + 2 * (p - 576)) = o;
        }
    }
    if (w == 7) {
#pragma unroll
        for (int mm = 0; mm < 8; mm++) { dpf4 o; o.x = tl[mm][0]; o.y = tl[mm][1]; o.z = tl[8 + mm][0]; o.w = tl[8 + mm][1]; *(dpf4*)(slot + 2 * (448 + 2 * g + 16 * mm)) = o; }
    }
    {
        dpf4 zz; zz.x = zz.y = zz.z = zz.w = 0.0f;
#pragma unroll
        for (int t4 = 0; t4 < 3; t4++) *(dpf4*)(slot + 2 * (576 + 2 * l + 128 * t4)) = zz;
        if (l < 32) *(dpf4*)(slot + 2 * (960 + 2 * l)) = zz;
    }
}

#define AACG_BR_LIVE    0x80000000u
#define AACG_BR_FLAG    0x00000001u
#define AACG_BR_NONE    127
struct quant_regs { dpi4 ql[2], qr[2]; unsigned mw[2][2]; };

template <bool NTL = false>
DP_DEVICE void quant_load(const void* coeffs, const aacg_band_meta* metas, uint32_t coef_block, uint32_t meta_block, int n_ch, quant_regs& r)
{
    const int lane = dp_lane();
    const int16_t* q0 = (const int16_t*)coeffs + (size_t)coef_block * 1024u;
    const aacg_band_meta* meta = metas + meta_block;
    const int16_t* q1 = q0 + (n_ch == 2 ? 1024 : 0);
    const aacg_band_meta* m1 = meta + (n_ch == 2 ? 1 : 0);
    const int b1 = lane + 64 < AACG_MAX_SECTIONS ? lane + 64 : AACG_MAX_SECTIONS - 1;
#pragma unroll
    for (int i = 0; i < 2; i++) {
        if (NTL) { r.ql[i] = dp_load_nt((const dpi4*)(q0 + 8 * lane + 512 * i)); r.qr[i] = dp_load_nt((const dpi4*)(q1 + 8 * lane + 512 * i)); }
        else {
        r.ql[i] = *(const dpi4*)(q0 + 8 * lane + 512 * i);
        r.qr[i] = *(const dpi4*)(q1 + 8 * lane + 512 * i);
        }
    }
    r.mw[0][0] = meta->band[lane]; r.mw[0][1] = meta->band[b1];
    r.mw[1][0] = m1->band[lane];   r.mw[1][1] = m1->band[b1];
}

struct chan_ctx {
    int cls;
    int max_sfb;
    unsigned gmap;
};

struct band_raw { dpf2 lng[2], sht; };
DP_DEVICE void band_raw_load(const float* tab, band_raw& r)
{
    const int lane = dp_lane();
    const unsigned char* bl = (const unsigned char*)(tab + AACG_TAB_OFF_BAND_LONG);
    const unsigned char* bs = (const unsigned char*)(tab + AACG_TAB_OFF_BAND_SHORT);
    r.lng[0] = *(const dpf2*)(bl + 8 * lane);
    r.lng[1] = *(const dpf2*)(bl + 8 * lane + 512);
    r.sht = *(const dpf2*)(bs + ((8 * lane) & 127));
}
DP_DEVICE void band_indices(const band_raw& r, const chan_ctx& cc, int (&idx)[4])
{
    const int lane = dp_lane();
#pragma unroll
    for (int i = 0; i < 2; i++) {
        const dpf2 m = cc.cls ? r.sht : r.lng[i];
        const int s0 = (int)(__builtin_bit_cast(unsigned, m.x) & 0xffu), s1 = (int)(__builtin_bit_cast(unsigned, m.y) & 0xffu);
        const int g = cc.cls ? (int)((cc.gmap >> (4 * ((lane >> 4) + 4 * i))) & 15u) : 0;
        idx[2 * i]     = s0 < cc.max_sfb ? g * cc.max_sfb + s0 : AACG_BR_NONE;
        idx[2 * i + 1] = s1 < cc.max_sfb ? g * cc.max_sfb + s1 : AACG_BR_NONE;
    }
}

template <int H0, int H1>
DP_DEVICE void prepare_bands(const quant_regs& r, const float* tab, bool two, bool ms_on, bool mask, float* bt)
{
    const int lane = dp_lane();
    unsigned* bw = (unsigned*)bt;
    const unsigned kCoded = 0x1FFEu;
    const unsigned kBelowNoise = 0x1FFFu;
    const unsigned kLiveR = two ? kCoded : 0u, kMsL = ms_on ? kBelowNoise : 0u;
    const unsigned kIs = two ? 0xC000u : 0u;
    const unsigned mask_u = mask ? 1u : 0u;
    float sl_in[2], sr_in[2];
#pragma unroll
    for (int h = H0; h < H1; h++) {
        sl_in[h] = tab[AACG_TAB_OFF_SF + (r.mw[0][h] & AACG_META_SF_MASK)];
        sr_in[h] = tab[AACG_TAB_OFF_SF + (r.mw[1][h] & AACG_META_SF_MASK)];
    }
#pragma unroll
    for (int h = H0; h < H1; h++) {
        const int b = lane + 64 * h;
        const bool coded = b < AACG_MAX_SECTIONS;
        const unsigned wl = coded ? r.mw[0][h] : 0u, wr = coded ? r.mw[1][h] : 0u;
        const unsigned tl = wl >> AACG_META_BT_SHIFT, tr = wr >> AACG_META_BT_SHIFT;
        const unsigned live_l = 0u - ((kCoded >> tl) & 1u), live_r = 0u - ((kLiveR >> tr) & 1u);
        const unsigned ms_used = (wl / AACG_META_MS_USED) & 1u;
        const unsigned ms = ms_used & (kMsL >> tl) & (kBelowNoise >> tr) & 1u;
        const unsigned is = (kIs >> tr) & 1u;
        const unsigned neg = ((0x4000u >> tr) ^ (mask_u & ms_used)) & 1u;
        const unsigned sl = __builtin_bit_cast(unsigned, sl_in[h]) ^ ((wl * (0x80000000u / AACG_META_NEGATE)) & 0x80000000u);
        const unsigned sr = __builtin_bit_cast(unsigned, sr_in[h]) ^ ((wr * (0x80000000u / AACG_META_NEGATE)) & 0x80000000u);
        dpf2 rl, rr;
        rl.x = __builtin_bit_cast(float, sl & live_l);
        rl.y = __builtin_bit_cast(float, (live_l & AACG_BR_LIVE) | ms);
        rr.x = __builtin_bit_cast(float, (sr & live_r) | ((sr ^ (neg << 31)) & (0u - is)));
        rr.y = __builtin_bit_cast(float, (live_r & AACG_BR_LIVE) | is);
        *(dpf2*)(bw + 2 * b) = rl;
        *(dpf2*)(bw + 256 + 2 * b) = rr;
    }
}

DP_DEVICE void dequant4(int iq0, float sf_eff, float z_eff, int p01, int p23, float (&x)[4], int& oor)
{
    oor |= dp_pk_add_u16(p01, 0x02000200) | dp_pk_add_u16(p23, 0x02000200);
    dpv2 a, b, sf, z;
    a[0] = dp_lds_read_f32(dp_mad4_i16_lo(p01, iq0)); a[1] = dp_lds_read_f32(dp_mad4_i16_hi(p01, iq0));
    b[0] = dp_lds_read_f32(dp_mad4_i16_lo(p23, iq0)); b[1] = dp_lds_read_f32(dp_mad4_i16_hi(p23, iq0));
    sf[0] = sf[1] = sf_eff; z[0] = z[1] = z_eff;
    a = dp_fma2(a, sf, z);
    b = dp_fma2(b, sf, z);
    x[0] = a[0]; x[1] = a[1]; x[2] = b[0]; x[3] = b[1];
}
#define AACG_OOR_MASK ((int)0xFC00FC00)

DP_DEVICE void dequant4_big(const aacg_tables* T, bool live, float sf, int p01, int p23, float (&x)[4])
{
    const int q[4] = {(int)(short)(p01 & 0xffff), p01 >> 16, (int)(short)(p23 & 0xffff), p23 >> 16};
#pragma unroll
    for (int e = 0; e < 4; e++) {
        const int a = q[e] < 0 ? -q[e] : q[e];
        if ((q[e] + 512) & ~1023) {
            const float v = T->iq[a > 8191 ? 8191 : a];
            x[e] = live ? (q[e] > 0 ? v : -v) * sf : 0.0f;
        }
    }
}

DP_DEVICE void wave_excl_scan2(int& v0, int& v1)
{
    const int lane = dp_lane();
    int in0 = v0, in1 = v1;
#pragma unroll
    for (int d = 1; d < 64; d <<= 1) {
        float t[2] = {__builtin_bit_cast(float, in0), __builtin_bit_cast(float, in1)};
        dp_shfl(t, (lane - d) & 63);
        if (lane >= d) { in0 += __builtin_bit_cast(int, t[0]); in1 += __builtin_bit_cast(int, t[1]); }
    }
    float tot[1] = {__builtin_bit_cast(float, in0)};
    dp_shfl(tot, 63);
    v0 = in0 - v0;
    v1 = in1 - v1 + __builtin_bit_cast(int, tot[0]);
}

DP_DEVICE void pns_channel(const aacg_pns_tables* T, const float* tab, const chan_ctx& cc, const unsigned (&mw)[2],
                           int* nb, float (&x)[16])
{
    const int lane = dp_lane();
    const uint16_t* swb = cc.cls ? T->swb_short : T->swb_long;
    auto group_len = [&](int g) { int n = 0; for (int w = 0; w < 8; w++) n += (cc.cls && ((cc.gmap >> (4 * w)) & 15u) == (unsigned)g) ? 1 : 0; return cc.cls ? n : 1; };
    int cnt[2]; bool noise[2];
#pragma unroll
    for (int h = 0; h < 2; h++) {
        const int b = lane + 64 * h;
        const unsigned wd = mw[h];
        noise[h] = b < AACG_MAX_SECTIONS && (int)(wd >> AACG_META_BT_SHIFT) == AACG_NOISE_BT && cc.max_sfb > 0;
        const int g = cc.max_sfb > 0 ? b / cc.max_sfb : 0, sfb = cc.max_sfb > 0 ? b % cc.max_sfb : 0;
        cnt[h] = noise[h] ? group_len(g) * ((int)swb[sfb + 1] - (int)swb[sfb]) : 0;
    }
    int first[2] = {cnt[0], cnt[1]};
    wave_excl_scan2(first[0], first[1]);
#pragma unroll
    for (int h = 0; h < 2; h++) {
        const int b = lane + 64 * h;
        nb[b] = noise[h] ? first[h] : -1;
        float sf = tab[AACG_TAB_OFF_SF + (mw[h] & AACG_META_SF_MASK)];
        if (mw[h] & AACG_META_NEGATE) sf = -sf;
        ((float*)nb)[128 + b] = sf;
    }
    dp_wave_sync();
    band_raw braw;
    band_raw_load(tab, braw);
    int idx[4];
    band_indices(braw, cc, idx);
#pragma unroll
    for (int k = 0; k < 4; k++) {
        const int i = k >> 1, h = k & 1;
        const int pos = 8 * lane + 512 * i + 4 * h;
        const int p_band = idx[k] == AACG_BR_NONE ? -1 : nb[idx[k]];
        if (p_band >= 0) {
            const int w = cc.cls ? pos >> 7 : 0;
            const int g = cc.cls ? (int)((cc.gmap >> (4 * w)) & 15u) : 0;
            int rank = 0;
            for (int v = 0; v < 8; v++) rank += (cc.cls && v < w && ((cc.gmap >> (4 * v)) & 15u) == (unsigned)g) ? 1 : 0;
            const int sfb = idx[k] - g * cc.max_sfb;
            const int width = (int)swb[sfb + 1] - (int)swb[sfb];
            const int pw = p_band + rank * width;
            const int k0 = (cc.cls ? (pos & 127) : pos) - (int)swb[sfb];
            const double energy = T->esum[pw + width] - T->esum[pw];
            const double scale = (double)((const float*)nb)[128 + idx[k]] / __builtin_sqrt(energy);
#pragma unroll
            for (int e = 0; e < 4; e++) x[4 * k + e] = (float)((double)T->rnd[(pw + k0 + e) & 1023] * scale);
        }
    }
    dp_wave_sync();
}

template <bool PNS = false>
DP_DEVICE void spectral_quant(const aacg_kparams& P, const float* tab, const unit_view& u, int n_ch,
                              const quant_regs& qreg, float* bt, float (&xl)[16], float (&xr)[16])
{
    chan_ctx ccL, ccR;
    ccL.cls = u.seq[0] == AACG_EIGHT_SHORT_SEQUENCE; ccL.max_sfb = u.max_sfb[0]; ccL.gmap = u.gmap[0];
    ccR.cls = u.seq[1] == AACG_EIGHT_SHORT_SEQUENCE; ccR.max_sfb = u.max_sfb[1]; ccR.gmap = u.gmap[1];

    const dpi4 (&ql)[2] = qreg.ql;
    const dpi4 (&qr)[2] = qreg.qr;
    const bool two = n_ch == 2;
    const bool ms_on = two && (u.flags & AACG_UNIT_COMMON_WINDOW) && (u.flags & AACG_UNIT_MASK_PRESENT);
    const bool mask  = (u.flags & AACG_UNIT_MASK_PRESENT) != 0;
    band_raw braw;
    band_raw_load(tab, braw);
    if (ccL.cls | ccR.cls) {
        dp_keep_branch();
        prepare_bands<0, 2>(qreg, tab, two, ms_on, mask, bt);
    } else {
        prepare_bands<0, 1>(qreg, tab, two, ms_on, mask, bt);
        dpf2 none; none.x = none.y = 0.0f;
        *(dpf2*)(bt + 2 * (64 + dp_lane())) = none;
        *(dpf2*)(bt + 256 + 2 * (64 + dp_lane())) = none;
    }
    int idxL[4], idxR[4];
    band_indices(braw, ccL, idxL);
#pragma unroll
    for (int k = 0; k < 4; k++) idxR[k] = idxL[k];
    if (ccR.cls != ccL.cls || ccR.max_sfb != ccL.max_sfb || ccR.gmap != ccL.gmap) {
        dp_keep_branch();
        band_indices(braw, ccR, idxR);
    }
    dp_wave_sync();

    dpf2 recL[4], recR[4];
#pragma unroll
    for (int k = 0; k < 4; k++) {
        recL[k] = *(const dpf2*)(bt + 2 * idxL[k]);
        recR[k] = *(const dpf2*)(bt + 256 + 2 * idxR[k]);
    }
    dp_lanes g_ms[4], g_is[4];
    bool  liveL[4], liveR[4], isR[4];
    float g_isc[4], sfL[4], sfR[4];
    int big = 0;
    const int iq0 = dp_lds_addr(tab + AACG_TAB_OFF_IQ_SMALL + 512);
#pragma unroll
    for (int k = 0; k < 4; k++) {
        const int i = k >> 1, h = k & 1;
        const unsigned fl = __builtin_bit_cast(unsigned, recL[k].y), fr = __builtin_bit_cast(unsigned, recR[k].y);
        g_ms[k] = dp_lanes_where((fl & AACG_BR_FLAG) != 0);
        g_is[k] = dp_lanes_where((fr & AACG_BR_FLAG) != 0);
        isR[k] = (fr & AACG_BR_FLAG) != 0;
        liveL[k] = (fl & AACG_BR_LIVE) != 0;
        liveR[k] = (fr & AACG_BR_LIVE) != 0;
        sfL[k] = recL[k].x;
        g_isc[k] = recR[k].x;
        sfR[k] = isR[k] ? 0.0f : recR[k].x;
        dequant4(iq0, sfL[k], __builtin_bit_cast(float, fl & AACG_BR_LIVE), h ? ql[i].z : ql[i].x, h ? ql[i].w : ql[i].y, *(float (*)[4])&xl[4 * k], big);
        dequant4(iq0, sfR[k], __builtin_bit_cast(float, fr & AACG_BR_LIVE), h ? qr[i].z : qr[i].x, h ? qr[i].w : qr[i].y, *(float (*)[4])&xr[4 * k], big);
    }

    if (dp_any((big & AACG_OOR_MASK) != 0)) {
#pragma unroll
        for (int k = 0; k < 4; k++) {
            const int i = k >> 1, h = k & 1;
            dequant4_big(P.tab, liveL[k], sfL[k], h ? ql[i].z : ql[i].x, h ? ql[i].w : ql[i].y, *(float (*)[4])&xl[4 * k]);
            dequant4_big(P.tab, liveR[k], sfR[k], h ? qr[i].z : qr[i].x, h ? qr[i].w : qr[i].y, *(float (*)[4])&xr[4 * k]);
        }
    }

    if (PNS && (u.flags & AACG_UNIT_HAS_PNS)) {
        pns_channel(P.pns, tab, ccL, qreg.mw[0], (int*)(bt + 512), xl);
        if (two) pns_channel(P.pns, tab, ccR, qreg.mw[1], (int*)(bt + 512), xr);
    }
    if (two) {
        if (dp_lanes_any(g_ms[0] | g_ms[1] | g_ms[2] | g_ms[3])) {
#pragma unroll
            for (int k = 0; k < 4; k++) {
                dpv2 a0 = v2(xl[4 * k], xl[4 * k + 1]), a1 = v2(xl[4 * k + 2], xl[4 * k + 3]);
                dpv2 b0 = v2(xr[4 * k], xr[4 * k + 1]), b1 = v2(xr[4 * k + 2], xr[4 * k + 3]);
                dp_sumdiff_where(g_ms[k], a0, a1, b0, b1);
                xl[4 * k] = a0[0]; xl[4 * k + 1] = a0[1]; xl[4 * k + 2] = a1[0]; xl[4 * k + 3] = a1[1];
                xr[4 * k] = b0[0]; xr[4 * k + 1] = b0[1]; xr[4 * k + 2] = b1[0]; xr[4 * k + 3] = b1[1];
            }
        }
        if (dp_lanes_any(g_is[0] | g_is[1] | g_is[2] | g_is[3])) {
#pragma unroll
            for (int k = 0; k < 4; k++) {
                const dpv2 l0 = v2(xl[4 * k], xl[4 * k + 1]), l1 = v2(xl[4 * k + 2], xl[4 * k + 3]);
                dpv2 r0 = v2(xr[4 * k], xr[4 * k + 1]), r1 = v2(xr[4 * k + 2], xr[4 * k + 3]);
                dp_scale_where(g_is[k], l0, l1, g_isc[k], r0, r1);
                xr[4 * k] = r0[0]; xr[4 * k + 1] = r0[1]; xr[4 * k + 2] = r1[0]; xr[4 * k + 3] = r1[1];
            }
        }
    }
    dp_wave_sync();
}

DP_DEVICE int stg(int k) { return k ^ (((k >> 6) & 3) << 3); }

DP_DEVICE void stage_nat8(const float (&x)[16], float* area)
{
    const int lane = dp_lane();
#pragma unroll
    for (int i = 0; i < 2; i++) {
        dpf4 a, b;
        a.x = x[8 * i]; a.y = x[8 * i + 1]; a.z = x[8 * i + 2]; a.w = x[8 * i + 3];
        b.x = x[8 * i + 4]; b.y = x[8 * i + 5]; b.z = x[8 * i + 6]; b.w = x[8 * i + 7];
        *(dpf4*)(area + 8 * lane + 512 * i) = a;
        *(dpf4*)(area + 8 * lane + 512 * i + 4) = b;
    }
}
DP_DEVICE void stage_pair_nat8(const float (&xl)[16], const float (&xr)[16], float* slot)
{
    const int lane = dp_lane();
#pragma unroll
    for (int i = 0; i < 2; i++) {
#pragma unroll
        for (int h = 0; h < 2; h++) {
            const int k = 4 * lane + 256 * i + 2 * h, e = 8 * i + 4 * h;
            dpf4 ev, od;
            ev.x = xl[e];     ev.y = xr[e];     ev.z = xl[e + 2]; ev.w = xr[e + 2];
            od.x = xl[e + 1]; od.y = xr[e + 1]; od.z = xl[e + 3]; od.w = xr[e + 3];
            *(dpf4*)(slot + 2 * stg(k)) = ev;
            *(dpf4*)(slot + 2 * (512 + stg(k))) = od;
        }
    }
}
DP_DEVICE void stage_pair_f32(const dpf4 (&xa)[4], const dpf4 (&xb)[4], float* slot)
{
    const int lane = dp_lane();
#pragma unroll
    for (int i = 0; i < 4; i++) {
        const int k = 2 * lane + 128 * i;
        dpf4 ev, od;
        ev.x = xa[i].x; ev.y = xb[i].x; ev.z = xa[i].z; ev.w = xb[i].z;
        od.x = xa[i].y; od.y = xb[i].y; od.z = xa[i].w; od.w = xb[i].w;
        *(dpf4*)(slot + 2 * stg(k)) = ev;
        *(dpf4*)(slot + 2 * (512 + stg(k))) = od;
    }
}

#define AACG_TNS_BLOCK 32
#define AACG_TNS_XCH_FLOATS(R) (2 * (R) * AACG_TNS_MAX_ORDER)

DP_DEVICE void tns_chunk_load(const float* blk, int inc, int c, float (&x)[4])
{
    const dpf4 t = *(const dpf4*)(blk + 4 * c * inc);
    if (inc > 0) { x[0] = t.x; x[1] = t.y; x[2] = t.z; x[3] = t.w; }
    else         { x[0] = t.w; x[1] = t.z; x[2] = t.y; x[3] = t.x; }
}
DP_DEVICE void tns_chunk_store(float* blk, int inc, int c, const float (&y)[4])
{
    dpf4 t;
    if (inc > 0) { t.x = y[0]; t.y = y[1]; t.z = y[2]; t.w = y[3]; }
    else         { t.w = y[0]; t.z = y[1]; t.y = y[2]; t.x = y[3]; }
    *(dpf4*)(blk + 4 * c * inc) = t;
}

template <int P, bool STORE>
DP_DEVICE void tns_run(float* blk, int inc, int chunks, int n_valid, const float (&lpc)[P], float (&h)[P])
{
#pragma unroll 1
    for (int c = 0; c < chunks; c++) {
        float x[4] = {0.0f, 0.0f, 0.0f, 0.0f}, y[4];
        if (4 * c < n_valid) tns_chunk_load(blk, inc, c, x);
#pragma unroll
        for (int j = 0; j < 4; j++) {
            float acc = x[j];
#pragma unroll
            for (int k = 1; k <= P; k++) acc = dp_fma(-lpc[k - 1], (k <= j) ? y[j - k] : h[k - j - 1], acc);
            y[j] = acc;
        }
        if (STORE && 4 * c < n_valid) tns_chunk_store(blk, inc, c, y);
#pragma unroll
        for (int k = P - 1; k >= 4; k--) h[k] = h[k - 4];
        h[0] = y[3]; h[1] = y[2]; h[2] = y[1]; h[3] = y[0];
    }
}

#define AACG_TNS_M_DOUBLES (3 * AACG_TNS_MAX_ORDER * AACG_TNS_MAX_ORDER)
DP_DEVICE const double* aacg_tns_m(const aacg_kparams& P) { return (const double*)(const void*)P.scratch; }
DP_DEVICE void tns_matrix_row(const float (&lpc)[AACG_TNS_MAX_ORDER], int r, double (&row)[AACG_TNS_MAX_ORDER])
{
    constexpr int P = AACG_TNS_MAX_ORDER, BL = 32;
#pragma unroll
    for (int k = 0; k < P; k++) row[k] = (k == r) ? 1.0 : 0.0;
#pragma unroll 2
    for (int step = 0; step < BL; step++) {
        const double w0 = row[0];
#pragma unroll
        for (int k = 0; k < P - 1; k++) row[k] = dp_fma(-w0, (double)lpc[k], row[k + 1]);
        row[P - 1] = -w0 * (double)lpc[P - 1];
    }
}
DP_DEVICE void tns_matrices_body(const aacg_dev_tns* recs, double* M, uint32_t n_records)
{
    constexpr int P = AACG_TNS_MAX_ORDER;
    const uint32_t rec = (uint32_t)dp_block() * AACG_WG_WAVES + (uint32_t)dp_wave();
    const int lane = dp_lane(), f = lane >> 4, r = lane & 15;
    if (rec >= n_records || f >= 3 || r >= P) return;
    const aacg_dev_tns* t = recs + rec;
    const int order = t->order[f];
    float lpc[P];
#pragma unroll
    for (int k = 0; k < P; k++) lpc[k] = (k < order) ? t->lpc[f][k] : 0.0f;
    double row[P];
    tns_matrix_row(lpc, r, row);
    double* dst = M + (size_t)rec * AACG_TNS_M_DOUBLES + (size_t)(f * P + r) * P;
#pragma unroll
    for (int k = 0; k < P; k++) dst[k] = row[k];
}

template <int R>
DP_DEVICE void tns_long_pass(float* slot, float* xch, const aacg_dev_tns* recA, const aacg_dev_tns* recB, int f, const double* mA, const double* mB)
{
    constexpr int P = AACG_TNS_MAX_ORDER, BL = AACG_TNS_BLOCK;
    const int lane = dp_lane(), half = lane >> 5, b = lane & 31;
    const int orderA = recA ? recA->order[f] : 0, orderB = recB ? recB->order[f] : 0;
    if (orderA <= 0 && orderB <= 0) return;
    const int sizeA = orderA > 0 ? recA->size[f] : 0, sizeB = orderB > 0 ? recB->size[f] : 0;
    const int n_steps = (((sizeA > sizeB ? sizeA : sizeB) + BL - 1) / BL) - 1;
    const aacg_dev_tns* rec = half ? recB : recA;
    const int order = half ? orderB : orderA, size = half ? sizeB : sizeA;
    const int start = order > 0 ? rec->start[f] : 0, inc = order > 0 ? rec->inc[f] : 1;
    float lpc[P];
#pragma unroll
    for (int k = 0; k < P; k++) lpc[k] = (k < order) ? rec->lpc[f][k] : 0.0f;
    float* area = slot + 1024 * half;
    float* cbuf = xch + AACG_TNS_XCH_FLOATS(R) / 2 * half;

    const int m0 = BL * b;
    const int n_valid = order > 0 ? (size - m0 < 0 ? 0 : (size - m0 > BL ? BL : size - m0)) : 0;
    float* blk = area + (inc > 0 ? start + m0 : start - m0 - 3);

    const int r16 = lane & 15;
    double row[P];
    const double* mrec = half ? mB : mA;
    {
        const bool have = mrec != nullptr && order > 0 && r16 < P;
        const double* src = have ? mrec + (size_t)(f * P + r16) * P : (mA ? mA : mB);
#pragma unroll
        for (int k = 0; k < P; k += 2) { const dpd2 t = *(const dpd2*)(src + k); row[k] = have ? t.x : 0.0; row[k + 1] = have ? t.y : 0.0; }
    }

    float c_own[P];
#pragma unroll
    for (int k = 0; k < P; k++) c_own[k] = 0.0f;
    tns_run<P, false>(blk, inc, BL / 4, n_valid, lpc, c_own);


    float s_in[P];
#pragma unroll
    for (int k = 0; k < P; k++) s_in[k] = 0.0f;
    float vmine = 0.0f;
#pragma unroll 1
    for (int g = 0; R * g <= n_steps; g++) {
        if (b / R == g) {
#pragma unroll
            for (int k = 0; k < P; k += 4) { dpf4 t; t.x = c_own[k]; t.y = c_own[k + 1]; t.z = c_own[k + 2]; t.w = c_own[k + 3]; *(dpf4*)(cbuf + P * (b % R) + k) = t; }
        }
        dp_wave_sync();
        float cs[R];
#pragma unroll
        for (int j = 0; j < R; j++) cs[j] = cbuf[P * j + (r16 < P ? r16 : 0)];
        dp_wave_sync();
#pragma unroll
        for (int j = 0; j < R; j++) {
            const int st = R * g + j;
            if (st <= n_steps) {
                double acc0 = (double)cs[j], acc1 = 0.0, acc2 = 0.0;
                if (st > 0) {
                    float f[P];
                    dp_row_gather12(vmine, f);
#pragma unroll
                    for (int k = 0; k < P; k++) s_in[k] = (b == st) ? f[k] : s_in[k];
#pragma unroll
                    for (int t = 0; t < P; t += 3) {
                        acc0 = dp_fma(row[t], (double)f[t], acc0);
                        acc1 = dp_fma(row[t + 1], (double)f[t + 1], acc1);
                        acc2 = dp_fma(row[t + 2], (double)f[t + 2], acc2);
                    }
                }
                vmine = (float)(acc0 + (acc1 + acc2));
            }
        }
    }

    tns_run<P, true>(blk, inc, BL / 4, n_valid, lpc, s_in);
    dp_wave_sync();
}

DP_DEVICE void tns_short_pass(float* slot, const aacg_dev_tns* recA, const aacg_dev_tns* recB, bool shortA, bool shortB)
{
    constexpr int P = 8;
    const int lane = dp_lane(), half = lane >> 5, w = lane & 31;
    const aacg_dev_tns* rec = half ? recB : recA;
    const bool mine = (half ? shortB : shortA) && rec != nullptr && w < 8;
    const int order = mine ? rec->order[w] : 0;
    const int size = order > 0 ? rec->size[w] : 0;
    const int start = order > 0 ? rec->start[w] : 0, inc = order > 0 ? rec->inc[w] : 1;
    float lpc[P];
#pragma unroll
    for (int k = 0; k < P; k++) lpc[k] = (k < order) ? rec->lpc[w][k] : 0.0f;
    float* blk = slot + 1024 * half + (inc > 0 ? start : start - 3);
    float h[P];
#pragma unroll
    for (int k = 0; k < P; k++) h[k] = 0.0f;
    if (dp_any(size > 0)) tns_run<P, true>(blk, inc, 32, size, lpc, h);
    dp_wave_sync();
}

template <int R>
DP_DEVICE void tns_unit(float* slot, float* xch, const aacg_dev_tns* rec0, const aacg_dev_tns* rec1, bool short0, bool short1,
                        const aacg_dev_tns* recs = nullptr, const double* M = nullptr)
{
    const aacg_dev_tns* l0 = short0 ? nullptr : rec0;
    const aacg_dev_tns* l1 = short1 ? nullptr : rec1;
    const double* m0 = (M && l0) ? M + (size_t)(l0 - recs) * AACG_TNS_M_DOUBLES : nullptr;
    const double* m1 = (M && l1) ? M + (size_t)(l1 - recs) * AACG_TNS_M_DOUBLES : nullptr;
    if (l0 || l1)
        for (int f = 0; f < 3; f++) tns_long_pass<R>(slot, xch, l0, l1, f, m0, m1);
    if ((short0 && rec0) || (short1 && rec1)) tns_short_pass(slot, rec0, rec1, short0, short1);
}

#define AACG_RUN_TNS_ROUND  3

#ifdef AACG_VM_F32
#define AACG_VM_KIND(kind) true
#else
#define AACG_VM_KIND(kind) ((kind) == AACG_INPUT_QUANT_I16)
#endif
template <bool VM>
DP_DEVICE void filter_unit(const float* tab, const unit_view& u, int n_ch, bool pair_path, bool want_head, float* slot,
                           float (&hx0)[8], float (&hy0)[8], float (&hx1)[8], float (&hy1)[8])
{
    chan_par p0, p1;
    p0.seq = u.seq[0]; p0.shape = u.shape[0]; p0.shape_prev = u.shape_prev[0];
    p1.seq = u.seq[1]; p1.shape = u.shape[1]; p1.shape_prev = u.shape_prev[1];
    const bool s0 = p0.seq == AACG_EIGHT_SHORT_SEQUENCE, s1 = p1.seq == AACG_EIGHT_SHORT_SEQUENCE;
    if (pair_path) {
        dpv2 hx[8], hy[8];
        if (s0) short_pair<VM>(tab, p0, slot, hx, hy);
        else    long_pair<VM>(tab, p0, want_head, slot, hx, hy);
#pragma unroll
        for (int m = 0; m < 8; m++) { hx0[m] = hx[m][0]; hx1[m] = hx[m][1]; hy0[m] = hy[m][0]; hy1[m] = hy[m][1]; }
        return;
    }
    {
        const chan_par cp[1] = {p0};
        float* const area[1] = {slot};
        float hx[1][8], hy[1][8];
        if (s0) short_channels<1, VM>(tab, cp, area, hx, hy);
        else    long_channels<1, VM>(tab, cp, want_head, area, hx, hy);
#pragma unroll
        for (int m = 0; m < 8; m++) { hx0[m] = hx[0][m]; hy0[m] = hy[0][m]; }
    }
    if (n_ch == 2) {
        const chan_par cp[1] = {p1};
        float* const area[1] = {slot + 1024};
        float hx[1][8], hy[1][8];
        if (s1) short_channels<1, VM>(tab, cp, area, hx, hy);
        else    long_channels<1, VM>(tab, cp, want_head, area, hx, hy);
#pragma unroll
        for (int m = 0; m < 8; m++) { hx1[m] = hx[0][m]; hy1[m] = hy[0][m]; }
        const int lane = dp_lane();
        dpf4 a[4], b[4];
        dp_wave_sync();
#pragma unroll
        for (int i = 0; i < 4; i++) { a[i] = *(const dpf4*)(slot + 4 * lane + 256 * i); b[i] = *(const dpf4*)(slot + 1024 + 4 * lane + 256 * i); }
// ... 78 lines not shown
#pragma unroll
    for (int k = 0; k < 2; k++) {
        if ((uint32_t)k < u.cpl_n) {
            const aacg_couple_job* job = AACG_CPL_JOBS(P) + (u.cpl_first + k);
            const float* src = AACG_CPL_SIDE(P) + (size_t)job->src * 1024u;
            pre.gain[k] = AACG_CPL_GAINS(P)[job->gain_off];
            pre.second[k] = job->dst != 0;
#pragma unroll
            for (int j = 0; j < 16; j++) pre.sv[k][j] = src[lane + 64 * j];
            pre.n = k + 1;
        }
    }
}

template <bool FROM_LDS, int OUT, bool CPL = false, bool SC1 = false>
DP_DEVICE void epilogue(const aacg_kparams& P, const cpl_prefetch& pre, const float* p0, const float* p1, const unit_view& u, int n_ch, int cls0, int cls1,
                        float* pcm_base_f32, const float (&hx0)[8], const float (&hy0)[8],
                        const float (&hx1)[8], const float (&hy1)[8], int lcol )
{
#pragma clang fp contract(off)
    const bool coupled = CPL && u.cpl_n > 0;
    typedef typename pcm_elem<OUT>::type elem;
    elem* pcm_base = (elem*)pcm_base_f32;
    const int lane = dp_lane(), w = lane >> 3, g = lane & 7;
    const int C = u.n_out_ch;
    elem* pcm = pcm_base + u.pcm_offset + u.channel;

    if (n_ch == 2 && C == 2 && !coupled && cls0 == cls1 && ((u.pcm_offset | (uint32_t)u.channel) & 3u) == 0) {
        if (!cls0) {
            dpf4 v[8];
#pragma unroll
            for (int m = 0; m < 8; m++) v[m] = incoming<FROM_LDS, SC1>(p0, p1, 2, 2 * lcol + 128 * m);
#pragma unroll
            for (int m = 0; m < 8; m++) {
                const int n = 2 * lcol + 128 * m;
                pcm_put4(pcm + 2 * n, v[m].x + hx0[m], v[m].y + hx1[m], v[m].z + hy0[m], v[m].w + hy1[m]);
            }
        } else {
#pragma unroll
            for (int m = 0; m < 8; m++) {
                if (w < 4 || (w == 4 && m < 4)) {
                    const int n = 448 + 128 * w + 2 * g + 16 * m;
                    const dpf4 v = incoming<FROM_LDS, SC1>(p0, p1, 2, n);
                    pcm_put4(pcm + 2 * n, v.x + hx0[m], v.y + hx1[m], v.z + hy0[m], v.w + hy1[m]);
                }
            }
#pragma unroll
            for (int t4 = 0; t4 < 4; t4++) {
                const int n = 2 * lane + 128 * t4;
                if (n < 448) {
                    const dpf4 v = incoming<FROM_LDS, SC1>(p0, p1, 2, n);
                    pcm_put4(pcm + 2 * n, v.x, v.y, v.z, v.w);
                }
            }
        }
        return;
    }

    if (FROM_LDS) {
        float* prev = const_cast<float*>(p0);
        overlap_add_in_place(prev, n_ch, cls0, cls1, lcol, hx0, hy0, hx1, hy1);
        dp_wave_sync();
        if (coupled) {
            float a[16], b[16];
#pragma unroll
            for (int j = 0; j < 16; j++) {
                const int n = lane + 64 * j;
                if (n_ch == 2) { const dpf2 lr = *(const dpf2*)(prev + 2 * n); a[j] = lr.x; b[j] = lr.y; }
                else           { a[j] = prev[n]; b[j] = 0.0f; }
            }
#pragma unroll
            for (int k = 0; k < 2; k++) {
                if (k < pre.n) {
#pragma unroll
                    for (int j = 0; j < 16; j++) { if (pre.second[k]) b[j] = dp_fma(pre.gain[k], pre.sv[k][j], b[j]); else a[j] = dp_fma(pre.gain[k], pre.sv[k][j], a[j]); }
                }
            }
            for (uint32_t k = (uint32_t)pre.n; k < u.cpl_n; k++) {
                const aacg_couple_job* job = AACG_CPL_JOBS(P) + (u.cpl_first + k);
                const float gain = AACG_CPL_GAINS(P)[job->gain_off];
                const float* src = AACG_CPL_SIDE(P) + (size_t)job->src * 1024u;
                const bool second = job->dst != 0;
                float sv[16];
#pragma unroll
                for (int j = 0; j < 16; j++) sv[j] = src[lane + 64 * j];
#pragma unroll
                for (int j = 0; j < 16; j++) { if (second) b[j] = dp_fma(gain, sv[j], b[j]); else a[j] = dp_fma(gain, sv[j], a[j]); }
            }
#pragma unroll
            for (int j = 0; j < 16; j++) {
                const int n = lane + 64 * j;
                if (n_ch == 2) pcm_put2(pcm + (size_t)n * C, a[j], b[j]); else pcm_put1(pcm + (size_t)n * C, a[j]);
            }
            return;
        }
        if (n_ch == 2) {
#pragma unroll
            for (int j = 0; j < 16; j++) {
                const int n = lane + 64 * j;
                const dpf2 lr = *(const dpf2*)(prev + 2 * n);
                pcm_put2(pcm + (size_t)n * C, lr.x, lr.y);
            }
        } else {
#pragma unroll
            for (int j = 0; j < 16; j++) {
                const int n = lane + 64 * j;
                pcm_put1(pcm + (size_t)n * C, prev[n]);
            }
        }
        return;
    }

    if (n_ch == 2 && cls0 == cls1 && !coupled) {
        if (!cls0) {
            dpf4 v[8];
#pragma unroll
            for (int m = 0; m < 8; m++) v[m] = incoming<FROM_LDS, SC1>(p0, p1, 2, 2 * lcol + 128 * m);
#pragma unroll
            for (int m = 0; m < 8; m++) {
                const int n = 2 * lcol + 128 * m;
                pcm_put2(pcm + (size_t)n * C, v[m].x + hx0[m], v[m].y + hx1[m]);
                pcm_put2(pcm + (size_t)(n + 1) * C, v[m].z + hy0[m], v[m].w + hy1[m]);
            }
        } else {
#pragma unroll
            for (int m = 0; m < 8; m++) {
                if (w < 4 || (w == 4 && m < 4)) {
                    const int n = 448 + 128 * w + 2 * g + 16 * m;
                    const dpf4 v = incoming<FROM_LDS, SC1>(p0, p1, 2, n);
                    pcm_put2(pcm + (size_t)n * C, v.x + hx0[m], v.y + hx1[m]);
                    pcm_put2(pcm + (size_t)(n + 1) * C, v.z + hy0[m], v.w + hy1[m]);
                }
            }
#pragma unroll
            for (int t4 = 0; t4 < 4; t4++) {
                const int n = 2 * lane + 128 * t4;
                if (n < 448) {
                    const dpf4 v = incoming<FROM_LDS, SC1>(p0, p1, 2, n);
                    pcm_put2(pcm + (size_t)n * C, v.x, v.y);
                    pcm_put2(pcm + (size_t)(n + 1) * C, v.z, v.w);
                }
            }
        }
        return;
    }

    if (coupled) {
#pragma unroll
        for (int c = 0; c < 2; c++) {
            if (c < n_ch) {
                elem* dst = pcm + c;
                const int cls = c ? cls1 : cls0;
                const float (&hx)[8] = c ? hx1 : hx0;
                const float (&hy)[8] = c ? hy1 : hy0;
                int pos[12]; bool ok[12]; float x[12], y[12];
#pragma unroll
                for (int i = 0; i < 12; i++) {
                    const int m = i & 7, t4 = i - 8;
                    if (i < 8) { pos[i] = cls ? 448 + 128 * w + 2 * g + 16 * m : 2 * lcol + 128 * m; ok[i] = !cls || w < 4 || (w == 4 && m < 4); }
                    else       { pos[i] = 2 * lane + 128 * t4; ok[i] = cls && pos[i] < 448; }
                    if (!ok[i]) pos[i] = 0;
                    const dpf4 v = incoming<FROM_LDS, SC1>(p0, p1, n_ch, pos[i]);
                    x[i] = (c ? v.y : v.x) + (i < 8 ? hx[m] : 0.0f);
                    y[i] = (c ? v.w : v.z) + (i < 8 ? hy[m] : 0.0f);
                }
                for (uint32_t k = 0; k < u.cpl_n; k++) {
                    const aacg_couple_job* job = AACG_CPL_JOBS(P) + (u.cpl_first + k);
                    if ((int)job->dst != c) continue;
                    const float gain = AACG_CPL_GAINS(P)[job->gain_off];
                    const float* src = AACG_CPL_SIDE(P) + (size_t)job->src * 1024u;
                    dpf2 sv[12];
#pragma unroll
                    for (int i = 0; i < 12; i++) sv[i] = *(const dpf2*)(src + pos[i]);
#pragma unroll
                    for (int i = 0; i < 12; i++) { x[i] = dp_fma(gain, sv[i].x, x[i]); y[i] = dp_fma(gain, sv[i].y, y[i]); }
                }
#pragma unroll
                for (int i = 0; i < 12; i++) {
                    if (ok[i]) { pcm_put1(dst + (size_t)pos[i] * C, x[i]); pcm_put1(dst + (size_t)(pos[i] + 1) * C, y[i]); }
                }
            }
        }
        return;
    }

#pragma unroll
    for (int c = 0; c < 2; c++) {
        if (c < n_ch) {
            elem* dst = pcm + c;
            const int cls = c ? cls1 : cls0;
            const float (&hx)[8] = c ? hx1 : hx0;
            const float (&hy)[8] = c ? hy1 : hy0;
            if (!cls) {
                dpf4 v[8];
#pragma unroll
                for (int m = 0; m < 8; m++) v[m] = incoming<FROM_LDS, SC1>(p0, p1, n_ch, 2 * lcol + 128 * m);
#pragma unroll
                for (int m = 0; m < 8; m++) {
                    const int n = 2 * lcol + 128 * m;
                    pcm_put1(dst + (size_t)n * C, (c ? v[m].y : v[m].x) + hx[m]);
                    pcm_put1(dst + (size_t)(n + 1) * C, (c ? v[m].w : v[m].z) + hy[m]);
                }
            } else {
#pragma unroll
                for (int m = 0; m < 8; m++) {
                    if (w < 4 || (w == 4 && m < 4)) {
                        const int n = 448 + 128 * w + 2 * g + 16 * m;
                        const dpf4 v = incoming<FROM_LDS, SC1>(p0, p1, n_ch, n);
                        pcm_put1(dst + (size_t)n * C, (c ? v.y : v.x) + hx[m]);
                        pcm_put1(dst + (size_t)(n + 1) * C, (c ? v.w : v.z) + hy[m]);
                    }
                }
#pragma unroll
                for (int t4 = 0; t4 < 4; t4++) {
                    const int n = 2 * lane + 128 * t4;
                    if (n < 448) {
                        const dpf4 v = incoming<FROM_LDS, SC1>(p0, p1, n_ch, n);
                        pcm_put1(dst + (size_t)n * C, c ? v.y : v.x);
                        pcm_put1(dst + (size_t)(n + 1) * C, c ? v.w : v.z);
                    }
                }
            }
        }
    }
}

DP_DEVICE void rv_publish_head(float* d0, float* d1, int n_ch, int cls0, int cls1, int lcol,
                               const float (&hx0)[8], const float (&hy0)[8], const float (&hx1)[8], const float (&hy1)[8])
{
    const int lane = dp_lane(), w = lane >> 3, g = lane & 7;
#pragma unroll
    for (int c = 0; c < 2; c++) {
        if (c < n_ch) {
            float* d = c ? d1 : d0;
            const int cls = c ? cls1 : cls0;
            const float (&hx)[8] = c ? hx1 : hx0;
            const float (&hy)[8] = c ? hy1 : hy0;
            if (!cls) {
#pragma unroll
                for (int m = 0; m < 8; m++) dp_g_store_f2(d + 2 * lcol + 128 * m, hx[m], hy[m]);
            } else {
#pragma unroll
                for (int m = 0; m < 8; m++)
                    if (w < 4 || (w == 4 && m < 4)) dp_g_store_f2(d + 448 + 128 * w + 2 * g + 16 * m, hx[m], hy[m]);
#pragma unroll
                for (int t4 = 0; t4 < 4; t4++) {
                    const int n = 2 * lane + 128 * t4;
                    if (n < 448) dp_g_store_f2(d + n, -0.0f, -0.0f);
                }
            }
        }
    }
}
DP_DEVICE void rv_publish_tails(const float* slot, int n_ch, float* d0, float* d1)
{
    const int lane = dp_lane();
#pragma unroll
    for (int i = 0; i < 8; i++) {
        const int n = 2 * lane + 128 * i;
        if (n_ch == 2) {
            const dpf4 a = *(const dpf4*)(slot + 2 * n);
            dp_g_store_f2(d0 + n, a.x, a.z);
            dp_g_store_f2(d1 + n, a.y, a.w);
        } else {
            const dpf2 a = *(const dpf2*)(slot + n);
            dp_g_store_f2(d0 + n, a.x, a.y);
        }
    }
}
template <int OUT>
DP_DEVICE void rv_finish_successor(typename pcm_elem<OUT>::type* pcm, int C, int n_ch, const float* slot, const float* h0, const float* h1)
{
#pragma clang fp contract(off)
    const int lane = dp_lane();
    if (n_ch == 2 && C == 2 && ((uintptr_t)pcm & (4u * sizeof(*pcm) - 1u)) == 0) {
        dpf2 hl[8], hr[8];
#pragma unroll
        for (int i = 0; i < 8; i++) { const int n = 2 * lane + 128 * i; hl[i] = dp_g_load_f2(h0 + n); hr[i] = dp_g_load_f2(h1 + n); }
#pragma unroll
        for (int i = 0; i < 8; i++) {
            const int n = 2 * lane + 128 * i;
            const dpf4 t = *(const dpf4*)(slot + 2 * n);
            pcm_put4(pcm + 2 * n, t.x + hl[i].x, t.y + hr[i].x, t.z + hl[i].y, t.w + hr[i].y);
        }
        return;
    }
#pragma unroll 4
    for (int j = 0; j < 16; j++) {
        const int n = lane + 64 * j;
        if (n_ch == 2) {
            const dpf2 t = *(const dpf2*)(slot + 2 * n);
            pcm_put2(pcm + (size_t)n * C, t.x + dp_g_load_f1(h0 + n), t.y + dp_g_load_f1(h1 + n));
        } else {
            pcm_put1(pcm + (size_t)n * C, slot[n] + dp_g_load_f1(h0 + n));
        }
    }
}

DP_DEVICE int ov_buffer(int rot, int add) { int r = rot + add; r = r >= AACG_OV_BUFFERS ? r - AACG_OV_BUFFERS : r; return r >= AACG_OV_BUFFERS ? r - AACG_OV_BUFFERS : r; }

#define AACG_RUN_XCH_FLOATS AACG_TNS_XCH_FLOATS(AACG_RUN_TNS_ROUND)
#define AACG_LDS_BYTES_F32_EX   (AACG_LDS_BYTES_F32 + 4 * AACG_WG_WAVES * AACG_RUN_XCH_FLOATS)
#define AACG_LDS_BYTES_QUANT_EX (AACG_LDS_BYTES_QUANT + 4 * AACG_WG_WAVES * AACG_RUN_XCH_FLOATS)
template <int KIND, int OUT = AACG_OUTPUT_F32, bool DD = false, bool EX = false, bool CPL = false, bool RV = false, bool NTL = false, bool PRE = false>
DP_DEVICE void imdct_run_body(const aacg_kparams& P, const aacg_rv_args* V = nullptr, const aacg_run* runs_pre = nullptr, const aacg_tables* tab_pre = nullptr, const aacg_rv_link* links_pre = nullptr,
                              const aacg_dev_unit* units_pre = nullptr, const void* coeffs_pre = nullptr, const aacg_band_meta* meta_pre = nullptr)
{
    const aacg_run* const k_runs = PRE ? runs_pre : P.runs;
    const aacg_tables* const k_tab = PRE ? tab_pre : P.tab;
    const aacg_dev_unit* const k_units = PRE ? units_pre : P.units;
    const void* const k_coeffs = PRE ? coeffs_pre : P.coeffs;
    const aacg_band_meta* const k_meta = PRE ? meta_pre : P.meta;
    const int TAB_FLOATS = (KIND == AACG_INPUT_QUANT_I16) ? AACG_TAB_QUANT_FLOATS : AACG_TAB_F32_FLOATS;
    const int lane = dp_lane(), wave = dp_wave();
    const aacg_run* run = k_runs + dp_block();
    float* lds = (float*)dp_lds_fixed<4 * AACG_LDS_FLOATS(TAB_FLOATS) + (EX ? 4 * AACG_WG_WAVES * AACG_RUN_XCH_FLOATS : 0)>();
    const float* tab = lds;
    float* slots = lds + AACG_TAB_SLOT_BASE(TAB_FLOATS);
    float* slot = slots + wave * AACG_SLOT_FLOATS;
    int* flags = (int*)(slots + AACG_WG_WAVES * AACG_SLOT_FLOATS);
    float* xch = EX ? (float*)(flags + AACG_WG_WAVES) + wave * AACG_RUN_XCH_FLOATS : nullptr;

    dp_su8 rh = dp_sload8(run, k_tab);
    dp_su4 lkw = dp_sload4(RV ? (const void*)((PRE ? links_pre : V->links) + dp_block()) : (const void*)run);
    unsigned w_unit = dp_sload1(run, (int)__builtin_offsetof(aacg_run, wave_unit) + 4 * wave);
    unsigned w_coef = dp_sload1(run, (int)__builtin_offsetof(aacg_run, wave_coef) + 4 * wave);
    unsigned w_meta = dp_sload1(run, (int)__builtin_offsetof(aacg_run, wave_meta) + 4 * wave);
    dpf4 tr0, tr1;
    stage_tables_load(k_tab, TAB_FLOATS, tr0, tr1);
    dp_swait(rh, lkw, w_unit, w_coef, w_meta);

    const int pred_unit = (int)rh[0], n_units = (int)rh[1];
    const bool run_is_last = rh[2] != 0;
    const int w_nch = (int)((rh[3] >> (2 * wave)) & 3u);
    const int run_ov0[2] = {(int)rh[4], (int)rh[5]}, run_rot[2] = {(int)rh[6], (int)rh[7]};
    const bool has_pred = !RV && pred_unit >= 0;
    aacg_rv_link lk; lk.link_in = lk.link_out = lk.succ_unit = -1; lk.reserved = 0;
    if (RV) { lk.link_in = (int)lkw[0]; lk.link_out = (int)lkw[1]; lk.succ_unit = (int)lkw[2]; }
    const bool xl = RV && V->xl_cells != nullptr;
    const bool hands_over = RV && wave == n_units - 1 && (lk.link_out >= 0 || xl);
    const bool hurry = hands_over;
#define AACG_OV_IN(c)  (run_ov0[c] + 1024 * ov_buffer(run_rot[c], P.flip))
#define AACG_OV_OUT(c) (run_ov0[c] + 1024 * ov_buffer(run_rot[c], P.flip + 1))
    const bool dd = DD && has_pred && n_units == AACG_WG_WAVES;
    const bool is_pred_wave = has_pred && !dd && wave == 0;
    const bool active = (has_pred && !dd) ? (wave == 0 || wave - 1 < n_units) : wave < n_units;
    const int n_pass = (DD && dd && wave == 0) ? 2 : 1;
    float* scratch = DD ? P.scratch + (size_t)dp_block() * AACG_SLOT_FLOATS : nullptr;

    float hx0[8], hy0[8], hx1[8], hy1[8];
    unit_view u = load_unit(k_units + dp_uniform((int)w_unit));
    if (NTL && !RV) {} else
    if (AACG_ABL(P, 64)) dp_setprio(0); else if (AACG_ABL(P, 32)) dp_setprio(1 - (wave >> 3)); else dp_setprio(hurry ? 3 : 3 - (wave >> 2));
    const unsigned long long t_start = AACG_ABL(P, 16) ? dp_clock() : 0;
    unsigned long long* trace = (!CPL && AACG_ABL(P, 16)) ? (unsigned long long*)P.spec_out + ((size_t)dp_block() * AACG_WG_WAVES + wave) * 8 : nullptr;
    if (trace && lane == 0) trace[0] = t_start;

    quant_regs qreg;
    dpf4 xa[4], xb[4];
    int n_ch = 0, cls0 = 0, cls1 = 0;
    bool pair_path = false;
    auto issue_loads = [&](uint32_t coef_block, uint32_t meta_block, int nch) {
        if (KIND == AACG_INPUT_QUANT_I16) quant_load<NTL>(k_coeffs, k_meta, coef_block, meta_block, nch, qreg);
        else {
            const float* xsrc = (const float*)k_coeffs + (size_t)coef_block * 1024u;
            const float* xsrc1 = xsrc + (nch == 2 ? 1024 : 0);
#pragma unroll
            for (int i = 0; i < 4; i++) {
                if (NTL) { xa[i] = dp_load_nt((const dpf4*)(xsrc + 4 * lane + 256 * i)); xb[i] = dp_load_nt((const dpf4*)(xsrc1 + 4 * lane + 256 * i)); }
                else     { xa[i] = *(const dpf4*)(xsrc + 4 * lane + 256 * i); xb[i] = *(const dpf4*)(xsrc1 + 4 * lane + 256 * i); }
            }
        }
    };
    auto save_tails = [&](float* d0, float* d1) {
#pragma unroll
        for (int i = 0; i < 4; i++) {
            const int n = 4 * lane + 256 * i;
            if (n_ch == 2) {
                const dpf4 a = *(const dpf4*)(slot + 2 * n), b = *(const dpf4*)(slot + 2 * n + 4);
                dpf4 l4, r4;
                l4.x = a.x; l4.y = a.z; l4.z = b.x; l4.w = b.z;
                r4.x = a.y; r4.y = a.w; r4.z = b.y; r4.w = b.w;
                *(dpf4*)(d0 + n) = l4;
                *(dpf4*)(d1 + n) = r4;
            } else {
                *(dpf4*)(d0 + n) = *(const dpf4*)(slot + n);
            }
        }
    };
    const bool early = wave < (KIND == AACG_INPUT_QUANT_I16 ? 2 : 4) || hurry || AACG_ABL(P, 128);
    if (early) issue_loads(w_coef, w_meta, w_nch);
    stage_tables_store(lds, TAB_FLOATS, tr0, tr1);
    if (lane == 0) flags[wave] = 0;
    dp_block_sync_lds();
    if (!early) issue_loads(w_coef, w_meta, w_nch);
    if (trace && lane == 0) trace[1] = dp_clock();
    n_ch = active ? u.n_ch : 0;
    cls0 = u.seq[0] == AACG_EIGHT_SHORT_SEQUENCE;
    cls1 = u.seq[1] == AACG_EIGHT_SHORT_SEQUENCE;
    pair_path = n_ch == 2 && u.seq[0] == u.seq[1] && u.shape[0] == u.shape[1] && u.shape_prev[0] == u.shape_prev[1];

    auto front = [&](bool want_head) {
        if (trace) { dp_vm_drain(); if (lane == 0) trace[6] = dp_clock(); }
        if (AACG_ABL(P, 1) && KIND != AACG_INPUT_QUANT_I16) {
#pragma unroll
            for (int m = 0; m < 8; m++) { hx0[m] = xa[m & 3].x; hy0[m] = xa[m & 3].y; hx1[m] = xb[m & 3].z; hy1[m] = xb[m & 3].w; }
            return;
        }
        if (KIND == AACG_INPUT_QUANT_I16) {
            float xl[16], xr[16];
            if (AACG_ABL(P, 8)) {
#pragma unroll
                for (int i = 0; i < 2; i++) {
                    xl[8 * i] = (float)qreg.ql[i].x; xl[8 * i + 1] = (float)qreg.ql[i].y; xl[8 * i + 2] = (float)qreg.ql[i].z; xl[8 * i + 3] = (float)qreg.ql[i].w;
                    xl[8 * i + 4] = xl[8 * i]; xl[8 * i + 5] = xl[8 * i + 1]; xl[8 * i + 6] = xl[8 * i + 2]; xl[8 * i + 7] = xl[8 * i + 3];
                    xr[8 * i] = (float)qreg.qr[i].x; xr[8 * i + 1] = (float)qreg.qr[i].y; xr[8 * i + 2] = (float)qreg.qr[i].z; xr[8 * i + 3] = (float)qreg.qr[i].w;
                    xr[8 * i + 4] = xr[8 * i]; xr[8 * i + 5] = xr[8 * i + 1]; xr[8 * i + 6] = xr[8 * i + 2]; xr[8 * i + 7] = xr[8 * i + 3];
                }
            } else
            spectral_quant<EX>(P, tab, u, n_ch, qreg, slot + 1024, xl, xr);
            if (EX && P.tns && (u.tns[0] || (n_ch == 2 && u.tns[1]))) {
                stage_nat8(xl, slot);
                if (n_ch == 2) stage_nat8(xr, slot + 1024);
                dp_wave_sync();
                tns_unit<AACG_RUN_TNS_ROUND>(slot, xch, u.tns[0] ? P.tns + u.tns_offset : nullptr, (n_ch == 2 && u.tns[1]) ? P.tns + u.tns_offset + 1 : nullptr,
                                             u.seq[0] == AACG_EIGHT_SHORT_SEQUENCE, u.seq[1] == AACG_EIGHT_SHORT_SEQUENCE, P.tns, aacg_tns_m(P));
#pragma unroll
                for (int i = 0; i < 2; i++) {
                    const dpf4 a = *(const dpf4*)(slot + 8 * lane + 512 * i), b = *(const dpf4*)(slot + 8 * lane + 512 * i + 4);
                    xl[8 * i] = a.x; xl[8 * i + 1] = a.y; xl[8 * i + 2] = a.z; xl[8 * i + 3] = a.w;
                    xl[8 * i + 4] = b.x; xl[8 * i + 5] = b.y; xl[8 * i + 6] = b.z; xl[8 * i + 7] = b.w;
                    const dpf4 c = *(const dpf4*)(slot + 1024 + 8 * lane + 512 * i), d = *(const dpf4*)(slot + 1024 + 8 * lane + 512 * i + 4);
                    xr[8 * i] = c.x; xr[8 * i + 1] = c.y; xr[8 * i + 2] = c.z; xr[8 * i + 3] = c.w;
                    xr[8 * i + 4] = d.x; xr[8 * i + 5] = d.y; xr[8 * i + 6] = d.z; xr[8 * i + 7] = d.w;
                }
                dp_wave_sync();
            }
            if (pair_path) stage_pair_nat8(xl, xr, slot);
            else { stage_nat8(xl, slot); if (n_ch == 2) stage_nat8(xr, slot + 1024); }
        } else {
            if (EX && P.tns && (u.tns[0] || (n_ch == 2 && u.tns[1]))) {
#pragma unroll
                for (int i = 0; i < 4; i++) {
                    *(dpf4*)(slot + 4 * lane + 256 * i) = xa[i];
                    if (n_ch == 2) *(dpf4*)(slot + 1024 + 4 * lane + 256 * i) = xb[i];
                }
                dp_wave_sync();
                tns_unit<AACG_RUN_TNS_ROUND>(slot, xch, u.tns[0] ? P.tns + u.tns_offset : nullptr, (n_ch == 2 && u.tns[1]) ? P.tns + u.tns_offset + 1 : nullptr,
                                             u.seq[0] == AACG_EIGHT_SHORT_SEQUENCE, u.seq[1] == AACG_EIGHT_SHORT_SEQUENCE, P.tns, aacg_tns_m(P));
#pragma unroll
                for (int i = 0; i < 4; i++) {
                    xa[i] = *(const dpf4*)(slot + 4 * lane + 256 * i);
                    xb[i] = *(const dpf4*)(slot + (n_ch == 2 ? 1024 : 0) + 4 * lane + 256 * i);
                }
                dp_wave_sync();
            }
            if (pair_path) stage_pair_f32(xa, xb, slot);
            else {
#pragma unroll
                for (int i = 0; i < 4; i++) {
                    *(dpf4*)(slot + 4 * lane + 256 * i) = xa[i];
                    if (n_ch == 2) *(dpf4*)(slot + 1024 + 4 * lane + 256 * i) = xb[i];
                }
            }
        }
        dp_wave_sync();
        if (trace && lane == 0) trace[2] = dp_clock();
        filter_unit<AACG_VM_KIND(KIND)>(tab, u, n_ch, pair_path, want_head, slot, hx0, hy0, hx1, hy1);
    };

    if (active) front(!is_pred_wave && n_pass == 1);
    if (DD && n_pass == 2) {
        dp_keep_branch();
        dp_wave_sync();
        save_tails(scratch, scratch + 1024);
        u = load_unit(P.units + dp_uniform(run->unit[0]));
        n_ch = u.n_ch;
        cls0 = u.seq[0] == AACG_EIGHT_SHORT_SEQUENCE;
        cls1 = u.seq[1] == AACG_EIGHT_SHORT_SEQUENCE;
        pair_path = n_ch == 2 && u.seq[0] == u.seq[1] && u.shape[0] == u.shape[1] && u.shape_prev[0] == u.shape_prev[1];
        issue_loads(u.coef_offset, u.meta_offset, u.n_ch);
        dp_wave_sync();
        front(true);
    }

    dp_wave_sync();
    if (lane == 0) dp_flag_set(&flags[wave], 1);
    if (trace && lane == 0) trace[3] = dp_clock();

    typedef typename pcm_elem<OUT>::type pcm_t;
    const unsigned long long rv_tag = RV ? V->epoch << 2 : 0ull;
    if (RV && hands_over && active) {
        dp_keep_branch();
        const bool cross = lk.link_out < 0;
        aacg_xl_cell* cell = cross ? V->xl_cells + ((run_ov0[0] >> 10) + ov_buffer(run_rot[0], P.flip + 1)) : nullptr;
        float* data = cross ? nullptr : V->data + (size_t)lk.link_out * AACG_RV_DATA_FLOATS;
        unsigned long long* st = cross ? &cell->state : V->state + (size_t)lk.link_out * AACG_RV_STATE_WORDS;
        float* t0 = cross ? P.overlap + AACG_OV_OUT(0) : data;
        float* t1 = cross ? P.overlap + AACG_OV_OUT(1) : data + 1024;
        const float* h0 = cross ? V->xl_head + AACG_OV_OUT(0) : data + 2048;
        const float* h1 = cross ? V->xl_head + AACG_OV_OUT(1) : data + 2048 + 1024;
        const unsigned long long seen = dp_first_u64(dp_g_load_u64(st));
        bool theirs = seen == (rv_tag | AACG_RV_HEAD);
        if (!theirs) {
            rv_publish_tails(slot, n_ch, t0, t1);
            dp_vm_drain();
            dp_wave_sync();
            bool won = true;
            if (lane == 0) won = dp_g_cas_u64(st, seen, rv_tag | AACG_RV_TAIL);
            theirs = dp_first_u64(won ? 0ull : 1ull) != 0ull;
        }
        if (theirs) {
            pcm_t* dst; int C;
            if (cross) {
                dst = (pcm_t*)(uintptr_t)dp_first_u64(dp_g_load_u64(&cell->pcm));
                C = dp_uniform((int)dp_g_load_u32(&cell->n_out_ch));
            } else {
                const unit_view su = load_unit(P.units + dp_uniform(lk.succ_unit));
                dst = (pcm_t*)P.pcm + su.pcm_offset + su.channel;
                C = su.n_out_ch;
            }
            rv_finish_successor<OUT>(dst, C, n_ch, slot, h0, h1);
        }
    }

    if (active && !is_pred_wave && AACG_ABL(P, 2)) {
        float acc = 0.0f;
#pragma unroll
        for (int m = 0; m < 8; m++) acc += hx0[m] + hy0[m] + hx1[m] + hy1[m];
        if (acc == 123456.789f) P.pcm[0] = acc;
    } else if (active && !is_pred_wave) {
        const int lcol = AACG_VM_KIND(KIND) ? long_col(lane) : lane;
        if (wave == 0) {
            const float* ov0 = n_pass == 2 ? scratch : P.overlap + AACG_OV_IN(0);
            const float* ov1 = n_pass == 2 ? scratch + 1024 : P.overlap + AACG_OV_IN(1);
            cpl_prefetch none; none.n = 0;
            const bool cross = xl && lk.link_in < 0 && V->epoch_in != 0ull;
            if (RV && (lk.link_in >= 0 || cross)) {
                dp_keep_branch();
                aacg_xl_cell* cell = cross ? V->xl_cells + ((run_ov0[0] >> 10) + ov_buffer(run_rot[0], P.flip)) : nullptr;
                float* data = cross ? nullptr : V->data + (size_t)lk.link_in * AACG_RV_DATA_FLOATS;
                unsigned long long* st = cross ? &cell->state : V->state + (size_t)lk.link_in * AACG_RV_STATE_WORDS;
                const float* t0 = cross ? P.overlap + AACG_OV_IN(0) : data;
                const float* t1 = cross ? P.overlap + AACG_OV_IN(1) : data + 1024;
                float* h0 = cross ? V->xl_head + AACG_OV_IN(0) : data + 2048;
                float* h1 = cross ? V->xl_head + AACG_OV_IN(1) : data + 2048 + 1024;
                const unsigned long long tag = cross ? V->epoch_in << 2 : rv_tag;
                const unsigned long long seen = dp_first_u64(dp_g_load_u64(st));
                bool theirs = seen == (tag | AACG_RV_TAIL);
                if (!theirs) {
                    rv_publish_head(h0, h1, n_ch, cls0, cls1, lcol, hx0, hy0, hx1, hy1);
                    if (cross && lane == 0) {
                        dp_g_store_u64(&cell->pcm, (unsigned long long)(uintptr_t)((pcm_t*)P.pcm + u.pcm_offset + u.channel));
                        dp_g_store_u32(&cell->n_out_ch, (unsigned)u.n_out_ch);
                    }
                    dp_vm_drain();
                    dp_wave_sync();
                    bool won = true;
                    if (lane == 0) won = dp_g_cas_u64(st, seen, tag | AACG_RV_HEAD);
                    theirs = dp_first_u64(won ? 0ull : 1ull) != 0ull;
                }
                if (theirs) epilogue<false, OUT, CPL, true>(P, none, t0, t1, u, n_ch, cls0, cls1, P.pcm, hx0, hy0, hx1, hy1, lcol);
            } else
            epilogue<false, OUT, CPL>(P, none, ov0, ov1, u, n_ch, cls0, cls1, P.pcm, hx0, hy0, hx1, hy1, lcol);
        } else {
            cpl_prefetch pre;
            couple_prefetch<CPL>(P, u, pre);
            dp_flag_wait(&flags[wave - 1], 1);
            if (trace && lane == 0) trace[4] = dp_clock();
            epilogue<true, OUT, CPL>(P, pre, slot - AACG_SLOT_FLOATS, slot - AACG_SLOT_FLOATS, u, n_ch, cls0, cls1, P.pcm, hx0, hy0, hx1, hy1, lcol);
        }
        if (trace && lane == 0) trace[5] = dp_clock();
        const int last_wave = (has_pred && !dd) ? n_units : n_units - 1;
        if (wave == last_wave && run_is_last && !xl)
            save_tails(P.overlap + AACG_OV_OUT(0), P.overlap + AACG_OV_OUT(1));
    }
    if (trace) {
        dp_vm_drain();
        if (lane == 0) trace[7] = ((unsigned long long)dp_cu_id() << 52) | (dp_clock() & 0xfffffffffffffull);
    }
}

#undef AACG_OV_IN
#undef AACG_OV_OUT

#define AACG_SPX_TAB_FLOATS  (AACG_TAB_QUANT_FLOATS - AACG_TAB_F32_FLOATS)
#define AACG_SPX_TNS_ROUND   4
#define AACG_SPX_XCH_FLOATS  AACG_TNS_XCH_FLOATS(AACG_SPX_TNS_ROUND)
#define AACG_SPX_WAVE_FLOATS (AACG_SLOT_FLOATS + AACG_SPX_XCH_FLOATS)
template <int KIND>
DP_DEVICE void spectral_ex_body(const aacg_kparams& P, int n_units)
{
    const int TAB_FLOATS = (KIND == AACG_INPUT_QUANT_I16) ? AACG_SPX_TAB_FLOATS : 0;
    const int lane = dp_lane(), wave = dp_wave();
    float* lds = (float*)dp_lds();
    const float* tab = lds - AACG_TAB_F32_FLOATS;
    float* slot = lds + TAB_FLOATS + wave * AACG_SPX_WAVE_FLOATS;
    float* xch = slot + AACG_SLOT_FLOATS;
    if (KIND == AACG_INPUT_QUANT_I16) {
        stage_tables((const aacg_tables*)((const float*)P.tab + AACG_TAB_F32_FLOATS), lds, AACG_SPX_TAB_FLOATS);
        dp_block_sync();
    }
    const int ui = dp_block() * AACG_WG_WAVES + wave;
    if (ui >= n_units) return;
    const unit_view u = load_unit(P.units + dp_uniform(ui));
    const int n_ch = u.n_ch;
    float xl[16], xr[16];
    if (KIND == AACG_INPUT_QUANT_I16) {
        quant_regs qreg;
        quant_load(P.coeffs, P.meta, u.coef_offset, u.meta_offset, n_ch, qreg);
        spectral_quant<true>(P, tab, u, n_ch, qreg, slot, xl, xr);
    } else {
        const float* x0 = (const float*)P.coeffs + (size_t)u.coef_offset * 1024u;
        const float* x1 = x0 + (n_ch == 2 ? 1024 : 0);
#pragma unroll
        for (int i = 0; i < 2; i++) {
            const dpf4 a = *(const dpf4*)(x0 + 8 * lane + 512 * i), b = *(const dpf4*)(x0 + 8 * lane + 512 * i + 4);
            const dpf4 c = *(const dpf4*)(x1 + 8 * lane + 512 * i), d = *(const dpf4*)(x1 + 8 * lane + 512 * i + 4);
            xl[8 * i] = a.x; xl[8 * i + 1] = a.y; xl[8 * i + 2] = a.z; xl[8 * i + 3] = a.w;
            xl[8 * i + 4] = b.x; xl[8 * i + 5] = b.y; xl[8 * i + 6] = b.z; xl[8 * i + 7] = b.w;
            xr[8 * i] = c.x; xr[8 * i + 1] = c.y; xr[8 * i + 2] = c.z; xr[8 * i + 3] = c.w;
            xr[8 * i + 4] = d.x; xr[8 * i + 5] = d.y; xr[8 * i + 6] = d.z; xr[8 * i + 7] = d.w;
        }
    }
    const bool tns0 = P.tns && u.tns[0], tns1 = P.tns && n_ch == 2 && u.tns[1];
    if (tns0 || tns1) {
        stage_nat8(xl, slot);
        if (n_ch == 2) stage_nat8(xr, slot + 1024);
        dp_wave_sync();
        tns_unit<AACG_SPX_TNS_ROUND>(slot, xch, tns0 ? P.tns + u.tns_offset : nullptr, tns1 ? P.tns + u.tns_offset + 1 : nullptr,
                 u.seq[0] == AACG_EIGHT_SHORT_SEQUENCE, u.seq[1] == AACG_EIGHT_SHORT_SEQUENCE, P.tns, aacg_tns_m(P));
#pragma unroll
        for (int i = 0; i < 2; i++) {
            const dpf4 a = *(const dpf4*)(slot + 8 * lane + 512 * i), b = *(const dpf4*)(slot + 8 * lane + 512 * i + 4);
            xl[8 * i] = a.x; xl[8 * i + 1] = a.y; xl[8 * i + 2] = a.z; xl[8 * i + 3] = a.w;
            xl[8 * i + 4] = b.x; xl[8 * i + 5] = b.y; xl[8 * i + 6] = b.z; xl[8 * i + 7] = b.w;
            const dpf4 c = *(const dpf4*)(slot + 1024 + 8 * lane + 512 * i), d = *(const dpf4*)(slot + 1024 + 8 * lane + 512 * i + 4);
            xr[8 * i] = c.x; xr[8 * i + 1] = c.y; xr[8 * i + 2] = c.z; xr[8 * i + 3] = c.w;
            xr[8 * i + 4] = d.x; xr[8 * i + 5] = d.y; xr[8 * i + 6] = d.z; xr[8 * i + 7] = d.w;
        }
    }
    float* out = P.spec_out + (size_t)u.coef_offset * 1024u;
#pragma unroll
    for (int i = 0; i < 2; i++) {
        dpf4 a, b;
        a.x = xl[8 * i]; a.y = xl[8 * i + 1]; a.z = xl[8 * i + 2]; a.w = xl[8 * i + 3];
        b.x = xl[8 * i + 4]; b.y = xl[8 * i + 5]; b.z = xl[8 * i + 6]; b.w = xl[8 * i + 7];
        *(dpf4*)(out + 8 * lane + 512 * i) = a;
        *(dpf4*)(out + 8 * lane + 512 * i + 4) = b;
        if (n_ch == 2) {
            a.x = xr[8 * i]; a.y = xr[8 * i + 1]; a.z = xr[8 * i + 2]; a.w = xr[8 * i + 3];
            b.x = xr[8 * i + 4]; b.y = xr[8 * i + 5]; b.z = xr[8 * i + 6]; b.w = xr[8 * i + 7];
            *(dpf4*)(out + 1024 + 8 * lane + 512 * i) = a;
            *(dpf4*)(out + 1024 + 8 * lane + 512 * i + 4) = b;
        }
    }
}

DP_DEVICE void couple_spec_body(const aacg_couple_params& Q, int waves_per_block)
{
    const int lane = dp_lane(), j = dp_block() * waves_per_block + dp_wave();
    if (j >= Q.n_jobs) return;
    const aacg_couple_job& job = Q.jobs[j];
    const unit_view u = load_unit(Q.units + dp_uniform((int)job.cce_unit));
    const int is_short = u.seq[0] == AACG_EIGHT_SHORT_SEQUENCE, max_sfb = u.max_sfb[0];
    const float* src = Q.spec + (size_t)job.src * 1024u;
    float* dst = Q.spec + (size_t)job.dst * 1024u;
    const float* gains = Q.gains + job.gain_off;
    const aacg_band_meta* m = Q.meta ? Q.meta + u.meta_offset : nullptr;
#pragma unroll 4
    for (int i = 0; i < 16; i++) {
        const int k = lane + 64 * i;
        const int sfb = is_short ? Q.tab->band_of_short[k & 127] : Q.tab->band_of_long[k];
        const int g = is_short ? (int)((u.gmap[0] >> (4 * (k >> 7))) & 15u) : 0;
        if (sfb < max_sfb) {
            const int idx = g * max_sfb + sfb;
            if (!m || (m->band[idx] >> AACG_META_BT_SHIFT) != AACG_ZERO_BT) dst[k] = dp_fma(gains[idx], src[k], dst[k]);
        }
    }
}

DP_DEVICE void couple_pcm_body(const aacg_couple_params& Q, int waves_per_block)
{
    const int lane = dp_lane(), j = dp_block() * waves_per_block + dp_wave();
    if (j >= Q.n_jobs) return;
    const aacg_couple_job& job = Q.jobs[j];
    const float gain = Q.gains[job.gain_off];
    const float* src = Q.side + (size_t)job.src * 1024u;
    float* dst = Q.pcm + job.dst;
    const size_t stride = job.stride;
#pragma unroll 4
    for (int i = 0; i < 16; i++) {
        const int n = lane + 64 * i;
        dst[n * stride] = dp_fma(gain, src[n], dst[n * stride]);
    }
}

DP_DEVICE void spectral_body(const aacg_kparams& P, int n_units)
{
    const int lane = dp_lane(), wave = dp_wave();
    float* lds = (float*)dp_lds();
    const float* tab = lds;
    float* bt = lds + AACG_TAB_QUANT_FLOATS + wave * 512;
    stage_tables(P.tab, lds, AACG_TAB_QUANT_FLOATS);
    dp_block_sync();
    const int ui = dp_block() * AACG_WG_WAVES + wave;
    if (ui >= n_units) return;
    const unit_view u = load_unit(P.units + dp_uniform(ui));
    const int n_ch = u.n_ch;
    float xl[16], xr[16];
    quant_regs qreg;
    quant_load(P.coeffs, P.meta, u.coef_offset, u.meta_offset, n_ch, qreg);
    spectral_quant(P, tab, u, n_ch, qreg, bt, xl, xr);
    float* out = P.spec_out + (size_t)u.coef_offset * 1024u;
#pragma unroll
    for (int i = 0; i < 2; i++) {
        dpf4 a, b;
        a.x = xl[8 * i]; a.y = xl[8 * i + 1]; a.z = xl[8 * i + 2]; a.w = xl[8 * i + 3];
        b.x = xl[8 * i + 4]; b.y = xl[8 * i + 5]; b.z = xl[8 * i + 6]; b.w = xl[8 * i + 7];
        *(dpf4*)(out + 8 * lane + 512 * i) = a;
        *(dpf4*)(out + 8 * lane + 512 * i + 4) = b;
        if (n_ch == 2) {
            a.x = xr[8 * i]; a.y = xr[8 * i + 1]; a.z = xr[8 * i + 2]; a.w = xr[8 * i + 3];
            b.x = xr[8 * i + 4]; b.y = xr[8 * i + 5]; b.z = xr[8 * i + 6]; b.w = xr[8 * i + 7];
            *(dpf4*)(out + 1024 + 8 * lane + 512 * i) = a;
            *(dpf4*)(out + 1024 + 8 * lane + 512 * i + 4) = b;
        }
    }
}

#endif
```

aac.js_amd/csrc/aacg_routes.h:

```cpp
#ifndef AACG_ROUTES_H
#define AACG_ROUTES_H

#include "aacg_device.h"

enum {
    AACG_RK_QUANT = 1,
    AACG_RK_I16   = 2,
    AACG_RK_DD    = 4,
    AACG_RK_EX    = 8,
    AACG_RK_CPL   = 16,
    AACG_RK_RV    = 32,
    AACG_RK_NT    = 64
};

struct aacg_run_kernel {
    unsigned    key;
    const char* name;
    const void* fn;
    bool preloaded = false;
};
#define AACG_RUN_KERNEL_PRE(name, ...) \
    extern "C" __global__ __launch_bounds__(AACG_WG_THREADS) \
    void name(const aacg_run* runs, const aacg_tables* tab, const aacg_rv_link* links, const aacg_dev_unit* units, const void* coeffs, \
              const aacg_band_meta* meta, const aacg_kparams P, const aacg_rv_args V) \
    { imdct_run_body<__VA_ARGS__, true>(P, &V, runs, tab, links, units, coeffs, meta); }

extern const aacg_run_kernel aacg_run_kernels_plain[];  extern const int aacg_run_kernels_plain_n;
extern const aacg_run_kernel aacg_run_kernels_rv[];     extern const int aacg_run_kernels_rv_n;
extern const aacg_run_kernel aacg_run_kernels_nt[];     extern const int aacg_run_kernels_nt_n;
extern const aacg_run_kernel aacg_run_kernels_ext[];    extern const int aacg_run_kernels_ext_n;
extern const aacg_run_kernel aacg_run_kernels_i16[];    extern const int aacg_run_kernels_i16_n;
extern const aacg_run_kernel aacg_run_kernels_exrun[];  extern const int aacg_run_kernels_exrun_n;
extern const aacg_run_kernel aacg_run_kernels_couple[]; extern const int aacg_run_kernels_couple_n;

enum { AACG_STAGE_NONE = 0, AACG_STAGE_SPECTRAL_EX = 1, AACG_STAGE_DEPENDENT_COUPLING = 2 };
struct aacg_route {
    int      stage;
    bool     stage_quant;
    bool     has_run;
    unsigned run_key;
    bool     rv;
    bool     has_side;
    unsigned side_key;
    bool     side_first;
    bool     couple_pcm;
    bool     overlappable;
};

#ifdef AACG_HOST_H
aacg_route aacg_pick_route(int input_kind, int output_kind, int debug_route, bool tracing, const aacg_plan_host& h, bool pipelined);
std::string aacg_run_kernel_name(unsigned key);
std::string aacg_route_names(const aacg_route& r, bool any_tns);

#define AACG_PIPE_MARK  2
#define AACG_PIPE_DEPTH(S) ((((AACG_OV_BUFFERS - 1 + (S)) / (S) - AACG_PIPE_MARK) / AACG_PIPE_MARK) * AACG_PIPE_MARK)
struct aacg_pipe_order {
    int     stream;
    int64_t sync_round;
    bool    marked;
    int64_t complete_upto;
};
#define AACG_PIPE_RING  8
aacg_pipe_order aacg_pipeline_order(uint64_t n, int streams);
int aacg_pipeline_streams(const aacg_plan_host& h, unsigned run_key);
#endif

#endif
```

Measured before the change: 366.1 million.

## Run quant rendezvous IMDCT kernel as eight-wave workgroups processing two units per wave

The quantized rendezvous run kernel now launches with half the waves, and each wave handles two units in sequence. Seven LDS slots are recycled and guarded by extra flags, and the next unit's coefficient loads are prefetched. The inverse-quant table held in LDS is trimmed to a smaller range, with a global-memory fallback for out-of-range values, so that two workgroups fit per CU. This trades more serial work per wave and extra flag synchronisation for higher occupancy and less LDS table staging per CU.

```diff
diff --git a/aac.js_amd/csrc/aacg_device.h b/aac.js_amd/csrc/aacg_device.h
--- a/aac.js_amd/csrc/aacg_device.h
+++ b/aac.js_amd/csrc/aacg_device.h
@@ -39,10 +39,17 @@
 #define AACG_TAB_OFF_BAND_LONG    (AACG_TAB_OFF_IQ_SMALL + 1024)
 #define AACG_TAB_OFF_BAND_SHORT   (AACG_TAB_OFF_BAND_LONG + 256)
 #define AACG_TAB_QUANT_FLOATS     (AACG_TAB_OFF_BAND_SHORT + 32)
+#define AACG_TAB_IQ_CUT(iqh)      (1024 - 2 * (iqh))
 
 #define AACG_SLOT_FLOATS  2048
 #define AACG_TAB_SLOT_BASE(tab_floats) (((tab_floats) + 127) & ~127)
 #define AACG_LDS_FLOATS(tab_floats) (AACG_TAB_SLOT_BASE(tab_floats) + AACG_WG_WAVES * AACG_SLOT_FLOATS + AACG_WG_WAVES)
+#define AACG_HALF_WAVES   8
+#define AACG_HALF_SLOTS   7
+#define AACG_HALF_IQH     256
+#define AACG_HALF_LDS_BYTES(tab_floats) (4 * (AACG_TAB_SLOT_BASE(tab_floats) + AACG_HALF_SLOTS * AACG_SLOT_FLOATS + 2 * AACG_WG_WAVES))
+#define AACG_HALF_LDS_BYTES_QUANT AACG_HALF_LDS_BYTES(AACG_TAB_QUANT_FLOATS - AACG_TAB_IQ_CUT(AACG_HALF_IQH))
+static_assert(AACG_HALF_LDS_BYTES_QUANT <= 81920, "two eight-wave run workgroups per CU");
 #define AACG_LDS_BYTES_F32    (4 * AACG_LDS_FLOATS(AACG_TAB_F32_FLOATS))
 #define AACG_LDS_BYTES_QUANT  (4 * AACG_LDS_FLOATS(AACG_TAB_QUANT_FLOATS))
 
diff --git a/aac.js_amd/csrc/aacg_engine.hip b/aac.js_amd/csrc/aacg_engine.hip
--- a/aac.js_amd/csrc/aacg_engine.hip
+++ b/aac.js_amd/csrc/aacg_engine.hip
@@ -331,7 +331,7 @@
     if (k->key & AACG_RK_RV) { v = *V; args[1] = &v; }
     const void *a_runs = p.runs, *a_tab = p.tab, *a_links = V ? V->links : nullptr, *a_units = p.units, *a_coeffs = p.coeffs, *a_meta = p.meta;
     if (k->preloaded) { args[0] = &a_runs; args[1] = &a_tab; args[2] = &a_links; args[3] = &a_units; args[4] = &a_coeffs; args[5] = &a_meta; args[6] = &p; args[7] = &v; }
-    const dim3 block(AACG_WG_THREADS);
+    const dim3 block(k->threads);
     if (stop) HIP_TRY(e, hipExtLaunchKernel(k->fn, dim3(blocks), block, args, 0, s, nullptr, stop, 0), AACG_ERR_NO_DEVICE);
     else      HIP_TRY(e, hipLaunchKernel(k->fn, dim3(blocks), block, args, 0, s), AACG_ERR_NO_DEVICE);
     return AACG_OK;
diff --git a/aac.js_amd/csrc/aacg_engine_rv.hip b/aac.js_amd/csrc/aacg_engine_rv.hip
--- a/aac.js_amd/csrc/aacg_engine_rv.hip
+++ b/aac.js_amd/csrc/aacg_engine_rv.hip
@@ -3,13 +3,13 @@
 #include "aacg_kernels.h"
 #include "aacg_routes.h"
 
-AACG_RUN_KERNEL_PRE(aacg_imdct_run_quant_rv, AACG_INPUT_QUANT_I16, AACG_OUTPUT_F32, false, false, false, true, false)
+AACG_RUN_KERNEL_PRE_HALF(aacg_imdct_run_quant_rv, AACG_INPUT_QUANT_I16, AACG_OUTPUT_F32, false, false, false, true, false)
 AACG_RUN_KERNEL_PRE(aacg_imdct_run_f32_rv, AACG_INPUT_SPEC_F32, AACG_OUTPUT_F32, false, false, false, true, false)
 AACG_RUN_KERNEL_PRE(aacg_imdct_run_quant_rv_nt, AACG_INPUT_QUANT_I16, AACG_OUTPUT_F32, false, false, false, true, true)
 AACG_RUN_KERNEL_PRE(aacg_imdct_run_f32_rv_nt, AACG_INPUT_SPEC_F32, AACG_OUTPUT_F32, false, false, false, true, true)
 
 const aacg_run_kernel aacg_run_kernels_rv[] = {
-    {AACG_RK_RV | AACG_RK_QUANT, "aacg_imdct_run_quant_rv", (const void*)aacg_imdct_run_quant_rv, true},
+    {AACG_RK_RV | AACG_RK_QUANT, "aacg_imdct_run_quant_rv", (const void*)aacg_imdct_run_quant_rv, true, AACG_HALF_WAVES * 64},
     {AACG_RK_RV, "aacg_imdct_run_f32_rv", (const void*)aacg_imdct_run_f32_rv, true},
     {AACG_RK_RV | AACG_RK_NT | AACG_RK_QUANT, "aacg_imdct_run_quant_rv_nt", (const void*)aacg_imdct_run_quant_rv_nt, true},
     {AACG_RK_RV | AACG_RK_NT, "aacg_imdct_run_f32_rv_nt", (const void*)aacg_imdct_run_f32_rv_nt, true}
diff --git a/aac.js_amd/csrc/aacg_kernels.h b/aac.js_amd/csrc/aacg_kernels.h
--- a/aac.js_amd/csrc/aacg_kernels.h
+++ b/aac.js_amd/csrc/aacg_kernels.h
@@ -1,5 +1,7 @@
 #ifndef AACG_KERNELS_H
 #define AACG_KERNELS_H
+
+#include <type_traits>
 
 #include "devport.h"
 #include "aacg_device.h"
@@ -121,6 +123,27 @@
     if (tid < n4) dst[tid] = t0;
     if (tid + AACG_WG_THREADS < n4) dst[tid + AACG_WG_THREADS] = t1;
 }
+DP_DEVICE int stage_tables_half_src(int i)
+{
+    const int iq4 = AACG_TAB_OFF_IQ_SMALL / 4, cut4 = AACG_TAB_IQ_CUT(AACG_HALF_IQH) / 4;
+    return i < iq4 ? i : i < iq4 + AACG_HALF_IQH / 2 ? i + cut4 / 2 : i + cut4;
+}
+DP_DEVICE void stage_tables_load_half(const aacg_tables* T, int n_floats, dpf4& t0, dpf4& t1, dpf4& t2)
+{
+    const dpf4* src = (const dpf4*)T;
+    const int n4 = n_floats >> 2, tid = dp_tid(), nt = AACG_HALF_WAVES * 64;
+    t0 = src[stage_tables_half_src(tid < n4 ? tid : n4 - 1)];
+    t1 = src[stage_tables_half_src(tid + nt < n4 ? tid + nt : n4 - 1)];
+    t2 = src[stage_tables_half_src(tid + 2 * nt < n4 ? tid + 2 * nt : n4 - 1)];
+}
+DP_DEVICE void stage_tables_store_half(float* lds, int n_floats, const dpf4& t0, const dpf4& t1, const dpf4& t2)
+{
+    dpf4* dst = (dpf4*)lds;
+    const int n4 = n_floats >> 2, tid = dp_tid(), nt = AACG_HALF_WAVES * 64;
+    if (tid < n4) dst[tid] = t0;
+    if (tid + nt < n4) dst[tid + nt] = t1;
+    if (tid + 2 * nt < n4) dst[tid + 2 * nt] = t2;
+}
 DP_DEVICE void stage_tables(const aacg_tables* T, float* lds, int n_floats)
 {
     dpf4 t0, t1;
@@ -761,11 +784,12 @@
 };
 
 struct band_raw { dpf2 lng[2], sht; };
+template <int IQH = 512>
 DP_DEVICE void band_raw_load(const float* tab, band_raw& r)
 {
     const int lane = dp_lane();
-    const unsigned char* bl = (const unsigned char*)(tab + AACG_TAB_OFF_BAND_LONG);
-    const unsigned char* bs = (const unsigned char*)(tab + AACG_TAB_OFF_BAND_SHORT);
+    const unsigned char* bl = (const unsigned char*)(tab + AACG_TAB_OFF_BAND_LONG - AACG_TAB_IQ_CUT(IQH));
+    const unsigned char* bs = (const unsigned char*)(tab + AACG_TAB_OFF_BAND_SHORT - AACG_TAB_IQ_CUT(IQH));
     r.lng[0] = *(const dpf2*)(bl + 8 * lane);
     r.lng[1] = *(const dpf2*)(bl + 8 * lane + 512);
     r.sht = *(const dpf2*)(bs + ((8 * lane) & 127));
@@ -822,9 +846,10 @@
     }
 }
 
+template <int IQH = 512>
 DP_DEVICE void dequant4(int iq0, float sf_eff, float z_eff, int p01, int p23, float (&x)[4], int& oor)
 {
-    oor |= dp_pk_add_u16(p01, 0x02000200) | dp_pk_add_u16(p23, 0x02000200);
+    oor |= dp_pk_add_u16(p01, IQH * 0x00010001) | dp_pk_add_u16(p23, IQH * 0x00010001);
     dpv2 a, b, sf, z;
     a[0] = dp_lds_read_f32(dp_mad4_i16_lo(p01, iq0)); a[1] = dp_lds_read_f32(dp_mad4_i16_hi(p01, iq0));
     b[0] = dp_lds_read_f32(dp_mad4_i16_lo(p23, iq0)); b[1] = dp_lds_read_f32(dp_mad4_i16_hi(p23, iq0));
@@ -833,15 +858,16 @@
     b = dp_fma2(b, sf, z);
     x[0] = a[0]; x[1] = a[1]; x[2] = b[0]; x[3] = b[1];
 }
-#define AACG_OOR_MASK ((int)0xFC00FC00)
-
+#define AACG_OOR_MASK(IQH) ((int)(0xFFFFFFFFu ^ ((2u * (IQH) - 1u) * 0x00010001u)))
+
+template <int IQH = 512>
 DP_DEVICE void dequant4_big(const aacg_tables* T, bool live, float sf, int p01, int p23, float (&x)[4])
 {
     const int q[4] = {(int)(short)(p01 & 0xffff), p01 >> 16, (int)(short)(p23 & 0xffff), p23 >> 16};
 #pragma unroll
     for (int e = 0; e < 4; e++) {
         const int a = q[e] < 0 ? -q[e] : q[e];
-        if ((q[e] + 512) & ~1023) {
+        if ((q[e] + IQH) & ~(2 * IQH - 1)) {
             const float v = T->iq[a > 8191 ? 8191 : a];
             x[e] = live ? (q[e] > 0 ? v : -v) * sf : 0.0f;
         }
@@ -917,7 +943,7 @@
     dp_wave_sync();
 }
 
-template <bool PNS = false>
+template <bool PNS = false, int IQH = 512>
 DP_DEVICE void spectral_quant(const aacg_kparams& P, const float* tab, const unit_view& u, int n_ch,
                               const quant_regs& qreg, float* bt, float (&xl)[16], float (&xr)[16])
 {
@@ -931,7 +957,7 @@
     const bool ms_on = two && (u.flags & AACG_UNIT_COMMON_WINDOW) && (u.flags & AACG_UNIT_MASK_PRESENT);
     const bool mask  = (u.flags & AACG_UNIT_MASK_PRESENT) != 0;
     band_raw braw;
-    band_raw_load(tab, braw);
+    band_raw_load<IQH>(tab, braw);
     if (ccL.cls | ccR.cls) {
         dp_keep_branch();
         prepare_bands<0, 2>(qreg, tab, two, ms_on, mask, bt);
@@ -961,7 +987,7 @@
     bool  liveL[4], liveR[4], isR[4];
     float g_isc[4], sfL[4], sfR[4];
     int big = 0;
-    const int iq0 = dp_lds_addr(tab + AACG_TAB_OFF_IQ_SMALL + 512);
+    const int iq0 = dp_lds_addr(tab + AACG_TAB_OFF_IQ_SMALL + IQH);
 #pragma unroll
     for (int k = 0; k < 4; k++) {
         const int i = k >> 1, h = k & 1;
@@ -974,16 +1000,16 @@
         sfL[k] = recL[k].x;
         g_isc[k] = recR[k].x;
         sfR[k] = isR[k] ? 0.0f : recR[k].x;
-        dequant4(iq0, sfL[k], __builtin_bit_cast(float, fl & AACG_BR_LIVE), h ? ql[i].z : ql[i].x, h ? ql[i].w : ql[i].y, *(float (*)[4])&xl[4 * k], big);
-        dequant4(iq0, sfR[k], __builtin_bit_cast(float, fr & AACG_BR_LIVE), h ? qr[i].z : qr[i].x, h ? qr[i].w : qr[i].y, *(float (*)[4])&xr[4 * k], big);
-    }
-
-    if (dp_any((big & AACG_OOR_MASK) != 0)) {
+        dequant4<IQH>(iq0, sfL[k], __builtin_bit_cast(float, fl & AACG_BR_LIVE), h ? ql[i].z : ql[i].x, h ? ql[i].w : ql[i].y, *(float (*)[4])&xl[4 * k], big);
+        dequant4<IQH>(iq0, sfR[k], __builtin_bit_cast(float, fr & AACG_BR_LIVE), h ? qr[i].z : qr[i].x, h ? qr[i].w : qr[i].y, *(float (*)[4])&xr[4 * k], big);
+    }
+
+    if (dp_any((big & AACG_OOR_MASK(IQH)) != 0)) {
 #pragma unroll
         for (int k = 0; k < 4; k++) {
             const int i = k >> 1, h = k & 1;
-            dequant4_big(P.tab, liveL[k], sfL[k], h ? ql[i].z : ql[i].x, h ? ql[i].w : ql[i].y, *(float (*)[4])&xl[4 * k]);
-            dequant4_big(P.tab, liveR[k], sfR[k], h ? qr[i].z : qr[i].x, h ? qr[i].w : qr[i].y, *(float (*)[4])&xr[4 * k]);
+            dequant4_big<IQH>(P.tab, liveL[k], sfL[k], h ? ql[i].z : ql[i].x, h ? ql[i].w : ql[i].y, *(float (*)[4])&xl[4 * k]);
+            dequant4_big<IQH>(P.tab, liveR[k], sfR[k], h ? qr[i].z : qr[i].x, h ? qr[i].w : qr[i].y, *(float (*)[4])&xr[4 * k]);
         }
     }
 
@@ -1668,23 +1694,28 @@
 #define AACG_RUN_XCH_FLOATS AACG_TNS_XCH_FLOATS(AACG_RUN_TNS_ROUND)
 #define AACG_LDS_BYTES_F32_EX   (AACG_LDS_BYTES_F32 + 4 * AACG_WG_WAVES * AACG_RUN_XCH_FLOATS)
 #define AACG_LDS_BYTES_QUANT_EX (AACG_LDS_BYTES_QUANT + 4 * AACG_WG_WAVES * AACG_RUN_XCH_FLOATS)
-template <int KIND, int OUT = AACG_OUTPUT_F32, bool DD = false, bool EX = false, bool CPL = false, bool RV = false, bool NTL = false, bool PRE = false>
+template <int KIND, int OUT = AACG_OUTPUT_F32, bool DD = false, bool EX = false, bool CPL = false, bool RV = false, bool NTL = false, bool PRE = false,
+          int NW = AACG_WG_WAVES>
 DP_DEVICE void imdct_run_body(const aacg_kparams& P, const aacg_rv_args* V = nullptr, const aacg_run* runs_pre = nullptr, const aacg_tables* tab_pre = nullptr, const aacg_rv_link* links_pre = nullptr,
                               const aacg_dev_unit* units_pre = nullptr, const void* coeffs_pre = nullptr, const aacg_band_meta* meta_pre = nullptr)
 {
+    constexpr bool HALF = NW != AACG_WG_WAVES;
+    static_assert(!HALF || (NW == AACG_HALF_WAVES && RV && !DD && !EX && !CPL), "eight-wave runs: the rendezvous kernels without optional stages only");
+    constexpr int TPW = AACG_WG_WAVES / NW;
+    constexpr int IQH = (HALF && KIND == AACG_INPUT_QUANT_I16) ? AACG_HALF_IQH : 512;
     const aacg_run* const k_runs = PRE ? runs_pre : P.runs;
     const aacg_tables* const k_tab = PRE ? tab_pre : P.tab;
     const aacg_dev_unit* const k_units = PRE ? units_pre : P.units;
     const void* const k_coeffs = PRE ? coeffs_pre : P.coeffs;
     const aacg_band_meta* const k_meta = PRE ? meta_pre : P.meta;
-    const int TAB_FLOATS = (KIND == AACG_INPUT_QUANT_I16) ? AACG_TAB_QUANT_FLOATS : AACG_TAB_F32_FLOATS;
+    const int TAB_FLOATS = (KIND == AACG_INPUT_QUANT_I16) ? AACG_TAB_QUANT_FLOATS - AACG_TAB_IQ_CUT(IQH) : AACG_TAB_F32_FLOATS;
     const int lane = dp_lane(), wave = dp_wave();
     const aacg_run* run = k_runs + dp_block();
-    float* lds = (float*)dp_lds_fixed<4 * AACG_LDS_FLOATS(TAB_FLOATS) + (EX ? 4 * AACG_WG_WAVES * AACG_RUN_XCH_FLOATS : 0)>();
+    float* lds = (float*)dp_lds_fixed<HALF ? AACG_HALF_LDS_BYTES(TAB_FLOATS) : 4 * AACG_LDS_FLOATS(TAB_FLOATS) + (EX ? 4 * AACG_WG_WAVES * AACG_RUN_XCH_FLOATS : 0)>();
     const float* tab = lds;
     float* slots = lds + AACG_TAB_SLOT_BASE(TAB_FLOATS);
-    float* slot = slots + wave * AACG_SLOT_FLOATS;
-    int* flags = (int*)(slots + AACG_WG_WAVES * AACG_SLOT_FLOATS);
+    float* slot = slots + (HALF ? wave % AACG_HALF_SLOTS : wave) * AACG_SLOT_FLOATS;
+    int* flags = (int*)(slots + (HALF ? AACG_HALF_SLOTS : AACG_WG_WAVES) * AACG_SLOT_FLOATS);
     float* xch = EX ? (float*)(flags + AACG_WG_WAVES) + wave * AACG_RUN_XCH_FLOATS : nullptr;
 
     dp_su8 rh = dp_sload8(run, k_tab);
@@ -1692,25 +1723,27 @@
     unsigned w_unit = dp_sload1(run, (int)__builtin_offsetof(aacg_run, wave_unit) + 4 * wave);
     unsigned w_coef = dp_sload1(run, (int)__builtin_offsetof(aacg_run, wave_coef) + 4 * wave);
     unsigned w_meta = dp_sload1(run, (int)__builtin_offsetof(aacg_run, wave_meta) + 4 * wave);
-    dpf4 tr0, tr1;
-    stage_tables_load(k_tab, TAB_FLOATS, tr0, tr1);
+    dpf4 tr0, tr1, tr2;
+    if (HALF) stage_tables_load_half(k_tab, TAB_FLOATS, tr0, tr1, tr2);
+    else      stage_tables_load(k_tab, TAB_FLOATS, tr0, tr1);
     dp_swait(rh, lkw, w_unit, w_coef, w_meta);
 
     const int pred_unit = (int)rh[0], n_units = (int)rh[1];
-    const bool run_is_last = rh[2] != 0;
-    const int w_nch = (int)((rh[3] >> (2 * wave)) & 3u);
-    const int run_ov0[2] = {(int)rh[4], (int)rh[5]}, run_rot[2] = {(int)rh[6], (int)rh[7]};
+    bool run_is_last = rh[2] != 0;
+    int w_nch = (int)((rh[3] >> (2 * wave)) & 3u);
+    int run_ov0[2] = {(int)rh[4], (int)rh[5]}, run_rot[2] = {(int)rh[6], (int)rh[7]};
     const bool has_pred = !RV && pred_unit >= 0;
     aacg_rv_link lk; lk.link_in = lk.link_out = lk.succ_unit = -1; lk.reserved = 0;
     if (RV) { lk.link_in = (int)lkw[0]; lk.link_out = (int)lkw[1]; lk.succ_unit = (int)lkw[2]; }
     const bool xl = RV && V->xl_cells != nullptr;
-    const bool hands_over = RV && wave == n_units - 1 && (lk.link_out >= 0 || xl);
+    int task = wave;
+    bool hands_over = RV && task == n_units - 1 && (lk.link_out >= 0 || xl);
     const bool hurry = hands_over;
 #define AACG_OV_IN(c)  (run_ov0[c] + 1024 * ov_buffer(run_rot[c], P.flip))
 #define AACG_OV_OUT(c) (run_ov0[c] + 1024 * ov_buffer(run_rot[c], P.flip + 1))
     const bool dd = DD && has_pred && n_units == AACG_WG_WAVES;
     const bool is_pred_wave = has_pred && !dd && wave == 0;
-    const bool active = (has_pred && !dd) ? (wave == 0 || wave - 1 < n_units) : wave < n_units;
+    bool active = (has_pred && !dd) ? (wave == 0 || wave - 1 < n_units) : wave < n_units;
     const int n_pass = (DD && dd && wave == 0) ? 2 : 1;
     float* scratch = DD ? P.scratch + (size_t)dp_block() * AACG_SLOT_FLOATS : nullptr;
 
@@ -1726,10 +1759,10 @@
     dpf4 xa[4], xb[4];
     int n_ch = 0, cls0 = 0, cls1 = 0;
     bool pair_path = false;
-    auto issue_loads = [&](uint32_t coef_block, uint32_t meta_block, int nch) {
-        if (KIND == AACG_INPUT_QUANT_I16) quant_load<NTL>(k_coeffs, k_meta, coef_block, meta_block, nch, qreg);
+    auto issue_loads = [&](uint32_t coef_block, uint32_t meta_block, int nch, const void* coeffs, const aacg_band_meta* metas) {
+        if (KIND == AACG_INPUT_QUANT_I16) quant_load<NTL>(coeffs, metas, coef_block, meta_block, nch, qreg);
         else {
-            const float* xsrc = (const float*)k_coeffs + (size_t)coef_block * 1024u;
+            const float* xsrc = (const float*)coeffs + (size_t)coef_block * 1024u;
             const float* xsrc1 = xsrc + (nch == 2 ? 1024 : 0);
 #pragma unroll
             for (int i = 0; i < 4; i++) {
@@ -1755,18 +1788,49 @@
         }
     };
     const bool early = wave < (KIND == AACG_INPUT_QUANT_I16 ? 2 : 4) || hurry || AACG_ABL(P, 128);
-    if (early) issue_loads(w_coef, w_meta, w_nch);
-    stage_tables_store(lds, TAB_FLOATS, tr0, tr1);
-    if (lane == 0) flags[wave] = 0;
+    if (early) issue_loads(w_coef, w_meta, w_nch, k_coeffs, k_meta);
+    if (HALF) stage_tables_store_half(lds, TAB_FLOATS, tr0, tr1, tr2);
+    else      stage_tables_store(lds, TAB_FLOATS, tr0, tr1);
+    if (lane == 0) {
+#pragma unroll
+        for (int j = 0; j < (HALF ? 2 * TPW : 1); j++) flags[wave + NW * j] = 0;
+    }
     dp_block_sync_lds();
-    if (!early) issue_loads(w_coef, w_meta, w_nch);
+    if (!early) issue_loads(w_coef, w_meta, w_nch, k_coeffs, k_meta);
     if (trace && lane == 0) trace[1] = dp_clock();
+    const int task2 = HALF ? wave + NW : 0;
+    auto next_loads = [&]() {
+        w_nch = (int)(((unsigned)dp_uniform((int)run->wave_nch) >> (2 * task2)) & 3u);
+        issue_loads((unsigned)dp_uniform((int)run->wave_coef[task2]), (unsigned)dp_uniform((int)run->wave_meta[task2]), w_nch, P.coeffs, P.meta);
+    };
+
+    auto do_task = [&](auto K) {
+    constexpr int k = decltype(K)::value;
+    if (k > 0) {
+        task = wave + NW * k;
+        slot = slots + (task % AACG_HALF_SLOTS) * AACG_SLOT_FLOATS;
+        active = task < n_units;
+        if (!active) return;
+        u = load_unit(P.units + dp_uniform(run->wave_unit[task2]));
+        run_is_last = dp_uniform(run->is_last) != 0;
+        for (int c = 0; c < 2; c++) { run_ov0[c] = dp_uniform(run->ov0[c]); run_rot[c] = dp_uniform(run->rot[c]); }
+        if (RV) {
+            const aacg_rv_link* lp = (PRE ? links_pre : V->links) + dp_block();
+            lk.link_in = dp_uniform(lp->link_in); lk.link_out = dp_uniform(lp->link_out); lk.succ_unit = dp_uniform(lp->succ_unit);
+        }
+        hands_over = RV && task == n_units - 1 && (lk.link_out >= 0 || xl);
+        if (!AACG_ABL(P, 64) && !AACG_ABL(P, 32)) dp_setprio(3);
+        if (trace) {
+            trace = (unsigned long long*)P.spec_out + ((size_t)dp_block() * AACG_WG_WAVES + task) * 8;
+            if (lane == 0) trace[0] = trace[1] = dp_clock();
+        }
+    }
     n_ch = active ? u.n_ch : 0;
     cls0 = u.seq[0] == AACG_EIGHT_SHORT_SEQUENCE;
     cls1 = u.seq[1] == AACG_EIGHT_SHORT_SEQUENCE;
     pair_path = n_ch == 2 && u.seq[0] == u.seq[1] && u.shape[0] == u.shape[1] && u.shape_prev[0] == u.shape_prev[1];
 
-    auto front = [&](bool want_head) {
+    auto front = [&](bool want_head, bool prefetch = false) {
         if (trace) { dp_vm_drain(); if (lane == 0) trace[6] = dp_clock(); }
         if (AACG_ABL(P, 1) && KIND != AACG_INPUT_QUANT_I16) {
 #pragma unroll
@@ -1784,7 +1848,7 @@
                     xr[8 * i + 4] = xr[8 * i]; xr[8 * i + 5] = xr[8 * i + 1]; xr[8 * i + 6] = xr[8 * i + 2]; xr[8 * i + 7] = xr[8 * i + 3];
                 }
             } else
-            spectral_quant<EX>(P, tab, u, n_ch, qreg, slot + 1024, xl, xr);
+            spectral_quant<EX, IQH>(P, tab, u, n_ch, qreg, slot + 1024, xl, xr);
             if (EX && P.tns && (u.tns[0] || (n_ch == 2 && u.tns[1]))) {
                 stage_nat8(xl, slot);
                 if (n_ch == 2) stage_nat8(xr, slot + 1024);
@@ -1833,9 +1897,11 @@
         dp_wave_sync();
         if (trace && lane == 0) trace[2] = dp_clock();
         filter_unit<AACG_VM_KIND(KIND)>(tab, u, n_ch, pair_path, want_head, slot, hx0, hy0, hx1, hy1);
+        if (HALF && prefetch) next_loads();
     };
 
-    if (active) front(!is_pred_wave && n_pass == 1);
+    if (HALF && active && task >= AACG_HALF_SLOTS) dp_flag_wait(&flags[AACG_WG_WAVES + task - AACG_HALF_SLOTS + 1], 1);
+    if (active) front(!is_pred_wave && n_pass == 1, k + 1 < TPW);
     if (DD && n_pass == 2) {
         dp_keep_branch();
         dp_wave_sync();
@@ -1845,13 +1911,13 @@
         cls0 = u.seq[0] == AACG_EIGHT_SHORT_SEQUENCE;
         cls1 = u.seq[1] == AACG_EIGHT_SHORT_SEQUENCE;
         pair_path = n_ch == 2 && u.seq[0] == u.seq[1] && u.shape[0] == u.shape[1] && u.shape_prev[0] == u.shape_prev[1];
-        issue_loads(u.coef_offset, u.meta_offset, u.n_ch);
+        issue_loads(u.coef_offset, u.meta_offset, u.n_ch, k_coeffs, k_meta);
         dp_wave_sync();
         front(true);
     }
 
     dp_wave_sync();
-    if (lane == 0) dp_flag_set(&flags[wave], 1);
+    if (lane == 0) dp_flag_set(&flags[task], 1);
     if (trace && lane == 0) trace[3] = dp_clock();
 
     typedef typename pcm_elem<OUT>::type pcm_t;
@@ -1897,7 +1963,7 @@
         if (acc == 123456.789f) P.pcm[0] = acc;
     } else if (active && !is_pred_wave) {
         const int lcol = AACG_VM_KIND(KIND) ? long_col(lane) : lane;
-        if (wave == 0) {
+        if (task == 0) {
             const float* ov0 = n_pass == 2 ? scratch : P.overlap + AACG_OV_IN(0);
             const float* ov1 = n_pass == 2 ? scratch + 1024 : P.overlap + AACG_OV_IN(1);
             cpl_prefetch none; none.n = 0;
@@ -1932,19 +1998,28 @@
         } else {
             cpl_prefetch pre;
             couple_prefetch<CPL>(P, u, pre);
-            dp_flag_wait(&flags[wave - 1], 1);
+            dp_flag_wait(&flags[task - 1], 1);
             if (trace && lane == 0) trace[4] = dp_clock();
-            epilogue<true, OUT, CPL>(P, pre, slot - AACG_SLOT_FLOATS, slot - AACG_SLOT_FLOATS, u, n_ch, cls0, cls1, P.pcm, hx0, hy0, hx1, hy1, lcol);
+            float* const pslot = HALF ? slots + ((task - 1) % AACG_HALF_SLOTS) * AACG_SLOT_FLOATS : slot - AACG_SLOT_FLOATS;
+            epilogue<true, OUT, CPL>(P, pre, pslot, pslot, u, n_ch, cls0, cls1, P.pcm, hx0, hy0, hx1, hy1, lcol);
         }
         if (trace && lane == 0) trace[5] = dp_clock();
         const int last_wave = (has_pred && !dd) ? n_units : n_units - 1;
-        if (wave == last_wave && run_is_last && !xl)
+        if (task == last_wave && run_is_last && !xl)
             save_tails(P.overlap + AACG_OV_OUT(0), P.overlap + AACG_OV_OUT(1));
+    }
+    if (HALF && active && task >= 1) {
+        if (AACG_ABL(P, 2)) dp_flag_wait(&flags[task - 1], 1);
+        dp_wave_sync();
+        if (lane == 0) dp_flag_set(&flags[AACG_WG_WAVES + task], 1);
     }
     if (trace) {
         dp_vm_drain();
         if (lane == 0) trace[7] = ((unsigned long long)dp_cu_id() << 52) | (dp_clock() & 0xfffffffffffffull);
     }
+    };
+    do_task(std::integral_constant<int, 0>());
+    if constexpr (TPW > 1) do_task(std::integral_constant<int, 1>());
 }
 
 #undef AACG_OV_IN
diff --git a/aac.js_amd/csrc/aacg_routes.h b/aac.js_amd/csrc/aacg_routes.h
--- a/aac.js_amd/csrc/aacg_routes.h
+++ b/aac.js_amd/csrc/aacg_routes.h
@@ -18,12 +18,18 @@
     const char* name;
     const void* fn;
     bool preloaded = false;
+    unsigned threads = AACG_WG_THREADS;
 };
 #define AACG_RUN_KERNEL_PRE(name, ...) \
     extern "C" __global__ __launch_bounds__(AACG_WG_THREADS) \
     void name(const aacg_run* runs, const aacg_tables* tab, const aacg_rv_link* links, const aacg_dev_unit* units, const void* coeffs, \
               const aacg_band_meta* meta, const aacg_kparams P, const aacg_rv_args V) \
     { imdct_run_body<__VA_ARGS__, true>(P, &V, runs, tab, links, units, coeffs, meta); }
+#define AACG_RUN_KERNEL_PRE_HALF(name, ...) \
+    extern "C" __global__ __launch_bounds__(AACG_HALF_WAVES * 64, 4) \
+    void name(const aacg_run* runs, const aacg_tables* tab, const aacg_rv_link* links, const aacg_dev_unit* units, const void* coeffs, \
+              const aacg_band_meta* meta, const aacg_kparams P, const aacg_rv_args V) \
+    { imdct_run_body<__VA_ARGS__, true, AACG_HALF_WAVES>(P, &V, runs, tab, links, units, coeffs, meta); }
 
 extern const aacg_run_kernel aacg_run_kernels_plain[];  extern const int aacg_run_kernels_plain_n;
 extern const aacg_run_kernel aacg_run_kernels_rv[];     extern const int aacg_run_kernels_rv_n;
```

After: 402.3 million, median of 6. 1.1x the previous value.
